# tqch/v-diffusion-torch

Measured on AMD Instinct MI355X. Metric: train_images_per_sec, higher is better.
Workload: dtype fp32 (bf16x3 split products in the tile-engine GEMMs)

## Files before the change

### include/vdiff_hip.h

```cpp
#ifndef VDIFF_HIP_H
#define VDIFF_HIP_H
#include <stddef.h>
#include <stdint.h>

#ifdef __cplusplus
extern "C" {
#endif

#define VD_VERSION 100

int         vd_version(void);
const char* vd_last_error(void);

int         vd_set_reserved_cus(int32_t n);
int         vd_reserved_cus(void);

int         vd_mfma_calibrate(float* sink, unsigned long long* stamps, int32_t blocks, int32_t iters, uint32_t seed, void* stream);

enum { VD_ROW = 0,
       VD_COL = 1,
       VD_IM2COL = 2 };

typedef struct vd_gemm_desc {
    const float* A; const float* B; float* C;
    const float* bias;
    const float* R;
    int32_t M, N, K;
    int32_t a_kind, b_kind;
    int64_t lda, ldb, ldc, ldr;
    int32_t batch, nh;
    int64_t sAb, sAh, sBb, sBh, sCb, sCh, sRb, sRh;
    float   alpha;
    int32_t accumulate;
    int32_t H, W, Cin;
    int32_t splitk;
    float*  ws; int64_t ws_bytes;
    int32_t tile;
    float*  colsum;
    int32_t colsum_accumulate;
    float*  stats;
    int32_t stats_hw;
    int64_t sBias;
} vd_gemm_desc;

int vd_gemm(const vd_gemm_desc* d, void* stream);
int vd_gemm_last_tile(void);
int vd_gemm_split_forms(void);
int vd_gemm_plan_tile(int32_t M, int32_t N, int32_t K, int32_t a_kind, int32_t b_kind, int32_t batch, int32_t tile, int32_t stats);
size_t vd_gemm_grouped_wgrad_ws_bytes(int32_t count, int32_t M, int32_t N, int32_t splitk);
int vd_gemm_grouped_wgrad_auto_split(int32_t count, int32_t M, int32_t N, int32_t K, int32_t min_slabs, int32_t max_slabs);
int vd_gemm_grouped_wgrad(const float* const* A, const float* const* B, float* const* C, float* const* colsum, int32_t count,
                          int32_t M, int32_t N, int32_t K, int64_t lda, int64_t ldb, int64_t ldc, int32_t splitk, float* ws, size_t ws_bytes,
                          void* stream);

int vd_conv3x3(const float* xin, int64_t ldx, const float* wpack, const float* bias,
               const float* res, int64_t ldres, float* y, int64_t ldy,
               int32_t nimg, int32_t H, int32_t W, int32_t Cin, int32_t Cout, int32_t accumulate,
               float* stats_part , void* stream);

int vd_conv3x3_wino_supported(int32_t nimg, int32_t H, int32_t W, int32_t Cin, int32_t Cout, int64_t ldx, int64_t ldy, int64_t ldres);
int vd_conv3x3_wino(const float* xin, int64_t ldx, const float* U, const float* bias, const float* res, int64_t ldres,
                    float* y, int64_t ldy, int32_t nimg, int32_t H, int32_t W, int32_t Cin, int32_t Cout,
                    float* stats_part, void* stream);
int vd_conv3x3_wgrad_wino_supported(int32_t nimg, int32_t H, int32_t W, int32_t Cin, int32_t Cout, int64_t ldx, int64_t lddy);
size_t vd_conv3x3_wgrad_wino_ws_bytes(int32_t nimg, int32_t H, int32_t W, int32_t Cin, int32_t Cout);
int vd_conv3x3_wgrad_wino(const float* xin, int64_t ldx, const float* dy, int64_t lddy, int32_t nimg, int32_t H, int32_t W,
                          int32_t Cin, int32_t Cout, float* dw_oihw, float* dbias, int32_t Cin_w, int32_t Cout_w,
                          int32_t accumulate, float* ws, size_t ws_bytes, void* stream);
int vd_conv3x3_wgrad_wino_phase(const float* xin, int64_t ldx, const float* dy, int64_t lddy, int32_t nimg, int32_t H, int32_t W,
                                int32_t Cin, int32_t Cout, float* dw_oihw, float* dbias, int32_t Cin_w, int32_t Cout_w,
                                int32_t accumulate, float* ws, size_t ws_bytes, int32_t phase, void* stream);
int vd_wino_last_kernel(void);
int vd_wino_wgrad_last_kernel(void);
#ifdef VD_PROBES
int vd_wino_set_probe(unsigned long long* buf);
int vd_wino43_set_probe(unsigned long long* buf);
int vd_gn_set_spin_probe(unsigned* buf);
#endif
int vd_wino_pack(const float* w_oihw, int32_t Cout, int32_t Cin, float* uf , float* ud , void* stream);
int vd_conv3x3_dgrad_wino43_supported(int32_t nimg, int32_t H, int32_t W, int32_t Cin, int32_t Cout, int64_t lddy, int64_t lddx);
size_t vd_wino43_u_floats(int32_t Cout, int32_t Cin);
int vd_conv3x3_dgrad_wino43(const float* dy, int64_t lddy, const float* U43, float* dx, int64_t lddx, int32_t nimg, int32_t H, int32_t W,
                            int32_t Cin, int32_t Cout, void* stream);
int vd_wino43_last_kernel(void);
int vd_wino43_pack(const float* w_oihw, int32_t Cout, int32_t Cin, float* U43, void* stream);
int vd_wino43_pack_batched(const int64_t* items_dev, int32_t n, int64_t total_blocks, void* stream);
int vd_conv3x3_wino43_preferred(int32_t nimg, int32_t H, int32_t W, int32_t N);
int vd_conv3x3_wino43_fwd_supported(int32_t nimg, int32_t H, int32_t W, int32_t Cin, int32_t Cout, int64_t ldx, int64_t ldy, int64_t ldres);
int vd_wino43_pack_fwd(const float* w_oihw, int32_t Cout, int32_t Cin, float* U43f, void* stream);
int vd_conv3x3_wino43_fwd_chunk_rows(int32_t H, int32_t W);
int vd_conv3x3_wino43_fwd(const float* xin, int64_t ldx, const float* U43f, const float* bias, const float* res, int64_t ldres, float* y,
                          int64_t ldy, int32_t nimg, int32_t H, int32_t W, int32_t Cin, int32_t Cout, float* stats_part, void* stream);
int vd_conv3x3_wgrad_wino43_supported(int32_t nimg, int32_t H, int32_t W, int32_t Cin, int32_t Cout, int64_t ldx, int64_t lddy);
size_t vd_conv3x3_wgrad_wino43_ws_bytes(int32_t nimg, int32_t H, int32_t W, int32_t Cin, int32_t Cout);
int vd_conv3x3_wgrad_wino43(const float* xin, int64_t ldx, const float* dy, int64_t lddy, int32_t nimg, int32_t H, int32_t W,
                            int32_t Cin, int32_t Cout, float* dw_oihw, float* dbias, int32_t Cin_w, int32_t Cout_w,
                            int32_t accumulate, float* ws, size_t ws_bytes, void* stream);
int vd_conv3x3_wgrad_wino43_phase(const float* xin, int64_t ldx, const float* dy, int64_t lddy, int32_t nimg, int32_t H, int32_t W,
                                  int32_t Cin, int32_t Cout, float* dw_oihw, float* dbias, int32_t Cin_w, int32_t Cout_w,
                                  int32_t accumulate, float* ws, size_t ws_bytes, int32_t phase, void* stream);
int vd_wino43_wgrad_last_kernel(void);

int vd_wino_pack_batched(const int64_t* items_dev, int32_t n, int64_t total_blocks, void* stream);

int vd_im2col3x3(const float* x, int64_t ldx, float* xc , int32_t nimg, int32_t H, int32_t W, int32_t C, void* stream);
int vd_tap_gather(const float* z, int64_t ldz, const float* bias, float* out, int64_t ldo, int32_t nimg, int32_t H, int32_t W, int32_t Cout, void* stream);
int vd_tap_spread(const float* dy, int64_t lddy, float* dz, int64_t ldz, int32_t nimg, int32_t H, int32_t W, int32_t Cout, void* stream);
int vd_thin_wgrad_finish(const float* g, int32_t Cout_w, int32_t Cin, int32_t Cin_w, float* dw_oihw, int32_t accumulate,
                         const float* colsum, int32_t cs_stride, int32_t cs_off, float* dbias, void* stream);

size_t vd_conv3x3_wgrad_ws_bytes(int32_t nimg, int32_t H, int32_t W, int32_t Cin, int32_t Cout);
int vd_conv3x3_wgrad(const float* xin, int64_t ldx, const float* dy, int64_t lddy,
                     int32_t nimg, int32_t H, int32_t W, int32_t Cin, int32_t Cout,
                     float* dw_oihw, float* dbias, int32_t Cin_w, int32_t Cout_w, int32_t accumulate,
                     float* ws, size_t ws_bytes, void* stream);
int vd_conv3x3_wgrad_phase(const float* xin, int64_t ldx, const float* dy, int64_t lddy,
                           int32_t nimg, int32_t H, int32_t W, int32_t Cin, int32_t Cout,
                           float* dw_oihw, float* dbias, int32_t Cin_w, int32_t Cout_w, int32_t accumulate,
                           float* ws, size_t ws_bytes, int32_t phase, void* stream);

int vd_pack_conv3x3(const float* w_oihw, int32_t Cout_w, int32_t Cin_w,
                    float* wf, int32_t Cin_p, float* wd, int32_t Cout_p, void* stream);
int vd_pack_conv3x3_batched(const int64_t* items_dev, int32_t n, int64_t total_blocks, void* stream);

enum { VD_RS_NONE = 0, VD_RS_DOWN = 1, VD_RS_UP = 2 };

size_t vd_gn_ws_bytes(int32_t nimg, int32_t HW, int32_t C);
int vd_gn_stats(const float* x, int64_t ldx, int32_t nimg, int32_t HW, int32_t C, int32_t G, float eps,
                float* stats, float* ws, size_t ws_bytes, void* stream);

int vd_gn_stats_from_partials(const float* part1, int32_t C1, int32_t chunks1, const float* part2, int32_t C2, int32_t chunks2,
                              int32_t nimg, int32_t HW, int32_t G, float eps, float* stats, void* stream);

int vd_gn_coef_from_partials(const float* part1, int32_t C1, int32_t chunks1, const float* part2, int32_t C2, int32_t chunks2,
                             int32_t nimg, int32_t HW, int32_t G, float eps, const float* gamma, const float* beta,
                             const float* film, float* coef, void* stream);

int vd_gn_apply(const float* x, int64_t ldx, const float* stats, const float* gamma, const float* beta,
                const float* film, int32_t act, float p_drop, uint64_t seed,
                int32_t resample, float* y, int64_t ldy,
                int32_t nimg, int32_t H, int32_t W, int32_t C, int32_t G, float* coef, void* stream);

int vd_gn_apply_from_partials(const float* x, int64_t ldx, const float* part1, int32_t C1, int32_t chunks1, const float* part2, int32_t C2,
                              int32_t chunks2, const float* gamma, const float* beta, const float* film, int32_t act, float p_drop,
                              uint64_t seed, int32_t resample, float* y, int64_t ldy, int32_t nimg, int32_t H, int32_t W, int32_t C,
                              int32_t G, float eps, float* coef, void* stream);

int vd_gn_apply_bwd(const float* dy, int64_t lddy, const float* x, int64_t ldx, const float* coef,
                    const float* gamma, const float* beta, const float* film, int32_t act, float p_drop, uint64_t seed,
                    int32_t resample, const float* add, int64_t ldadd, float* dx, int64_t lddx, int32_t accumulate_dx,
                    float* dfilm, float* dgamma, float* dbeta, int32_t accumulate_params,
                    int32_t nimg, int32_t H, int32_t W, int32_t C, int32_t G,
                    float* ws, size_t ws_bytes, void* stream);
int vd_gn_bwd_last_kernel(void);
int vd_gn_apply_bwd_keep(const float* dy, int64_t lddy, const float* x, int64_t ldx, const float* coef, const float* gamma,
                         const float* beta, const float* film, int32_t act, float p_drop, uint64_t seed, int32_t resample,
                         const float* add, int64_t ldadd, float* dx, int64_t lddx, int32_t accumulate_dx, float* dfilm, float* pgb_keep,
                         int32_t nimg, int32_t H, int32_t W, int32_t C, int32_t G, float* ws, size_t ws_bytes, void* stream);
int vd_gn_param_sums_batched(const int64_t* items_dev, int32_t n, int64_t total_blocks, void* stream);

size_t vd_colsum_ws_bytes(int64_t M, int32_t N);
int vd_colsum(const float* x, int64_t ldx, int64_t M, int32_t N, float* out, int32_t accumulate,
              float* ws, size_t ws_bytes, void* stream);
int vd_axpby(const float* x, int64_t ldx, float alpha, float* y, int64_t ldy, float beta, int64_t rows, int32_t C, void* stream);
int vd_silu(const float* x, float* y, int64_t n, void* stream);
int vd_silu_bwd(const float* x, const float* dy, float* dx, int64_t n, int32_t accumulate, void* stream);
int vd_softmax_rows(float* s, int64_t rows, int32_t L, void* stream);
int vd_softmax_rows_bwd(const float* p, float* dp, int64_t rows, int32_t L, float alpha, void* stream);

int vd_attn_supported(int32_t L, int32_t hd, int32_t backward);
int vd_attn_fwd(const float* q, const float* k, const float* v, int64_t ld, float* o, int64_t ldo, float* lse, int32_t B,
                int32_t nh, int32_t L, int32_t hd, float scale, void* stream);
int vd_attn_bwd(const float* q, const float* k, const float* v, int64_t ld, const float* o, int64_t ldo, const float* dout,
                int64_t lddo, const float* lse, float* delta, float* dq, float* dk, float* dv, int64_t ldd, int32_t B,
                int32_t nh, int32_t L, int32_t hd, float scale, void* stream);
int vd_attn_bwd_phase(const float* q, const float* k, const float* v, int64_t ld, const float* o, int64_t ldo, const float* dout,
                      int64_t lddo, const float* lse, float* delta, float* dq, float* dk, float* dv, int64_t ldd, int32_t B,
                      int32_t nh, int32_t L, int32_t hd, float scale, int32_t phase, void* stream);

int vd_nchw_to_nhwc(const float* x, float* y, int32_t nimg, int32_t C, int32_t H, int32_t W, int64_t ldy, void* stream);
int vd_nhwc_to_nchw(const float* x, int64_t ldx, float* y, int32_t nimg, int32_t C, int32_t H, int32_t W, void* stream);

int vd_images_to_uint8_hwc(const float* x_nchw, uint8_t* out_hwc, int32_t n, int32_t C, int32_t HW, void* stream);
int vd_images_from_uint8_hwc(const uint8_t* in_hwc, const uint8_t* flip, float* out_nchw, int32_t n, int32_t C,
// ... 114 lines not shown
```

### v-diffusion-torch_amd/csrc/common.h

```cpp
#pragma once
#include <hip/hip_runtime.h>
#include <stdint.h>
#include <stdio.h>
#include "../../include/vdiff_hip.h"

typedef float f32x4 __attribute__((ext_vector_type(4)));
typedef float f32x16 __attribute__((ext_vector_type(16)));

typedef float f32x2 __attribute__((ext_vector_type(2)));

#ifdef VD_PROBES
constexpr bool VD_PROBE_BUILD = true;
#else
constexpr bool VD_PROBE_BUILD = false;
#endif

void vd_set_error(const char* fmt, ...);
int vd_cu_count(void);
int vd_persistent_cus(void);
int vd_gemm_grouped_wgrad_kblk(const float* const* A, const float* const* B, float* const* C, float* const* colsum, int32_t count, int32_t M,
                               int32_t N, int32_t K, int64_t lda, int64_t ldb, int64_t ldc, int32_t splitk, float* ws, size_t ws_bytes,
                               void* stream, int64_t a_kblk, int64_t b_kblk, int32_t slabs_only);
int vd_gemm_grouped_wgrad_used_slabs(int32_t count, int32_t M, int32_t N, int32_t K, int32_t splitk);
extern thread_local int vd_g_last_tile;
inline int vd_tile_code(bool tr, bool spl, int kt, int bm, int bn) {
    return ((((tr ? 1 : 0) + (spl ? 2 : 0)) * 100 + kt) * 1000 + bm) * 1000 + bn;
}

#define VD_REQUIRE(cond, ...)                                   \
    do { if (!(cond)) { vd_set_error(__VA_ARGS__); return 1; } } while (0)

#define VD_LAUNCH_CHECK(name)                                                            \
    do { hipError_t e_ = hipGetLastError();                                              \
         if (e_ != hipSuccess) { vd_set_error("%s: %s", name, hipGetErrorString(e_)); return 2; } } while (0)

static inline bool vd_aligned16(const void* p) { return (reinterpret_cast<uintptr_t>(p) & 15) == 0; }

__device__ __forceinline__ float vd_sigmoid(float x) { return __builtin_amdgcn_rcpf(1.0f + __expf(-x)); }

__device__ __forceinline__ void vd_philox4(uint64_t seed, uint64_t ctr, uint32_t out[4]) {
    uint32_t k0 = (uint32_t)seed, k1 = (uint32_t)(seed >> 32);
    uint32_t c0 = (uint32_t)ctr, c1 = (uint32_t)(ctr >> 32), c2 = 0x243F6A88u, c3 = 0x85A308D3u;
#pragma unroll
    for (int r = 0; r < 10; ++r) {
        uint64_t p0 = (uint64_t)0xD2511F53u * c0, p1 = (uint64_t)0xCD9E8D57u * c2;
        uint32_t n0 = (uint32_t)(p1 >> 32) ^ c1 ^ k0, n2 = (uint32_t)(p0 >> 32) ^ c3 ^ k1;
        c1 = (uint32_t)p1; c3 = (uint32_t)p0; c0 = n0; c2 = n2;
        k0 += 0x9E3779B9u; k1 += 0xBB67AE85u;
    }
    out[0] = c0; out[1] = c1; out[2] = c2; out[3] = c3;
}
__device__ __forceinline__ f32x4 vd_dropout_scale4(uint64_t seed, uint64_t vec_index, float p) {
    uint32_t r[4];
    vd_philox4(seed, vec_index, r);
    const float inv = 1.0f / (1.0f - p);
    f32x4 m;
#pragma unroll
    for (int j = 0; j < 4; ++j) m[j] = ((r[j] >> 8) * (1.0f / 16777216.0f) >= p) ? inv : 0.0f;
    return m;
}
```

### v-diffusion-torch_amd/csrc/gemm.hip

```cpp
#include "common.h"
#include <math.h>
#include <stdlib.h>
#include <type_traits>

namespace {

constexpr int KT = 32;
#ifndef VD_GEMM_SPLIT_DEFAULT
#define VD_GEMM_SPLIT_DEFAULT 1
#endif

struct GemmArgs {
    const float* A; const float* B; float* C; const float* bias; const float* R;
    int M, N, K;
    long long lda, ldb, ldc, ldr;
    int nh;
    long long sAb, sAh, sBb, sBh, sCb, sCh, sRb, sRh;
    float alpha; int accumulate;
    int H, W, Cin;
    int kt_total, kt_per_split;
    long long slab_stride;
    float* colsum; int colsum_accumulate;
    int probe;
    float* stats; int stats_hw;
// ... 343 lines not shown
__device__ __forceinline__ void gemm_dma_body(const GemmArgs& p, const std::conditional_t<GROUPED, GroupPtrs, NoGroup>& gp) {
    constexpr int NBUF = 2;
    __shared__ __attribute__((aligned(1024))) float smem[NBUF * (BM + BN) * KT];
    constexpr int MT = BM / 64, NT = BN / 64;
    constexpr int AIT = BM * KT / 1024, BIT = BN * KT / 1024;
    constexpr int A_LPR = BM / 4, B_LPR = BN / 4;
    constexpr int A_RPP = 64 / A_LPR, B_RPP = 64 / B_LPR;
    constexpr int RLPR = KT / 4, RRPP = 64 / RLPR;
    constexpr bool A2 = (AK == VD_COL) && (MT == 2);
    constexpr bool B2 = (BK != VD_ROW) && (NT == 2 || NT == 4);
    typedef float f32x2 __attribute__((ext_vector_type(2)));
    typedef std::conditional_t<NT == 4, f32x4, f32x2> f32xNT;
    static_assert(NT <= 2 || (SPL && KT == 16 && !SPLITK && !GROUPED && AK != VD_IM2COL && BK != VD_IM2COL),
                  "256-column tiles: split-operand KT = 16 forms of plain / batched launches only");

    const int tid = threadIdx.x, lane = tid & 63;
    const int wave = __builtin_amdgcn_readfirstlane(tid >> 6);
    const int li = lane & 31, lh = lane >> 5;
    const int wm = (wave >> 1) * (BM / 2), wn = (wave & 1) * (BN / 2);
    int tbx = blockIdx.x, tby = blockIdx.y, tbz = blockIdx.z;
    {
        const unsigned T = gridDim.x * gridDim.y * gridDim.z;
        const unsigned lin = (blockIdx.z * gridDim.y + blockIdx.y) * gridDim.x + blockIdx.x;
        if (T >= 16) {
            const unsigned q = T / 8, r = T % 8, xcd = lin % 8, slot = lin / 8;
            const unsigned t = (xcd < r ? xcd * (q + 1) : r * (q + 1) + (xcd - r) * q) + slot;
            tbx = t % gridDim.x; tby = (t / gridDim.x) % gridDim.y; tbz = t / (gridDim.x * gridDim.y);
        }
    }
    const int m0 = tby * BM;
    int n0 = tbx * BN;
    int tapN = 0, ci0 = 0;
    if (BK == VD_IM2COL) {
        const int cchN = (p.Cin + BN - 1) / BN;
        tapN = tbx / cchN;
        ci0 = (tbx % cchN) * BN;
        n0 = tapN * p.Cin + ci0;
    }
    const float* A = p.A;
    const float* B = p.B;
    float* C = p.C;
    const float* R = p.R;
    const float* biasp = p.bias;
    int kt_begin = 0, kt_end = p.kt_total;
    if (SPLITK) {
        int slab = tbz;
        if constexpr (GROUPED) {
            const int e = tbz / p.group_S;
            slab = tbz - e * p.group_S;
            A = gp.A[e];
            B = gp.B[e];
        }
        kt_begin = slab * p.kt_per_split;
        kt_end = min(kt_begin + p.kt_per_split, p.kt_total);
        C += (long long)tbz * p.slab_stride;
    } else {
        const int zb = tbz / p.nh, zh = tbz % p.nh;
        A += zb * p.sAb + zh * p.sAh;
        B += zb * p.sBb + zh * p.sBh;
        C += zb * p.sCb + zh * p.sCh;
        if (R) R += zb * p.sRb + zh * p.sRh;
        if (biasp) biasp += zb * p.sBias;
    }

    unsigned voA[AIT], voB[BIT];
    unsigned mkA[AIT];
    int kcA[AIT], kcB[BIT];
    int by[BIT], bx[BIT];
    int tapA = (AK == VD_IM2COL) ? kt_begin % 9 : 0, ccA = (AK == VD_IM2COL) ? kt_begin / 9 : 0;
    const int kinc_x = (BK == VD_IM2COL) ? KT % p.W : 0, kinc_y = (BK == VD_IM2COL) ? KT / p.W : 0;
#pragma unroll
    for (int j = 0; j < AIT; ++j) {
        const int q = j * 4 + wave;
        if (AK == VD_COL) {
            const int kk = q * A_RPP + lane / A_LPR, cm = (lane % A_LPR) * 4;
            const int rowoff = (GROUPED && p.a_kblk) ? (kk >> 4) * (int)p.a_kblk + (kk & 15) * (int)p.lda : kk * (int)p.lda;
            voA[j] = (m0 + cm < p.M) ? (unsigned)(rowoff + cm) * 4u : OOB;
            kcA[j] = kk; mkA[j] = 0;
        } else {
            const int row = q * RRPP + lane / RLPR;
            const int c = (lane % RLPR) ^ swz_of<KT>(row);
            const int m = m0 + row;
            kcA[j] = c * 4;
            voA[j] = (m < p.M) ? (unsigned)(row * (int)p.lda + c * 4) * 4u : OOB;
            unsigned mk = 0;
            if (AK == VD_IM2COL) {
                int y, x;
                pix_yx(p, m, y, x);
                const unsigned xm = (x > 0 ? 1u : 0u) | 2u | (x < p.W - 1 ? 4u : 0u);
                mk = (y > 0 ? xm : 0u) | (xm << 3) | (y < p.H - 1 ? xm << 6 : 0u);
            }
            mkA[j] = mk;
        }
    }
#pragma unroll
    for (int j = 0; j < BIT; ++j) {
        const int q = j * 4 + wave;
        if (BK == VD_ROW) {
            const int row = q * RRPP + lane / RLPR;
            const int c = (lane % RLPR) ^ swz_of<KT>(row);
            kcB[j] = c * 4;
            voB[j] = (n0 + row < p.N) ? (unsigned)(row * (int)p.ldb + c * 4) * 4u : OOB;
            by[j] = bx[j] = 0;
        } else {
            const int kk = q * B_RPP + lane / B_LPR, cn = (lane % B_LPR) * 4;
            kcB[j] = kk;
            const bool ok = (BK == VD_IM2COL) ? (ci0 + cn < p.Cin) : (n0 + cn < p.N);
            const int rowoff = (GROUPED && BK == VD_COL && p.b_kblk) ? (kk >> 4) * (int)p.b_kblk + (kk & 15) * (int)p.ldb : kk * (int)p.ldb;
            voB[j] = ok ? (unsigned)(rowoff + cn) * 4u : OOB;
            if (BK == VD_IM2COL) pix_yx(p, kt_begin * KT + kk, by[j], bx[j]);
            else by[j] = bx[j] = 0;
        }
    }
    const float* Ablk = (AK == VD_COL) ? A + m0 : A + (long long)m0 * p.lda;
    const float* Bblk = (BK == VD_ROW) ? B + (long long)n0 * p.ldb : ((BK == VD_COL) ? B + n0 : B + ci0);
    const long long tapoffB = (BK == VD_IM2COL) ? (long long)((tapN / 3 - 1) * p.W + (tapN % 3 - 1)) * p.ldb : 0;

#ifndef VD_ISSUE_IN
#define VD_ISSUE_IN 2
#endif
    constexpr bool ISSUE_IN = VD_ISSUE_IN == 2 ? (AK == VD_COL) : (VD_ISSUE_IN == 1);
    struct Prep { const float* pA; const float* pB; unsigned vA[AIT], vB[BIT]; };
    auto prep_tiles = [&](int kt, Prep& P) {
        {
            const int tap = tapA, c0 = ccA * KT;
            long long aoff;
            int kwidth;
            if (AK == VD_IM2COL) { aoff = (long long)((tap / 3 - 1) * p.W + (tap % 3 - 1)) * p.lda + c0; kwidth = p.Cin - c0; }
            else if (AK == VD_ROW) { aoff = (long long)kt * KT; kwidth = p.K - kt * KT; }
            else { aoff = (GROUPED && p.a_kblk) ? (long long)kt * (KT / 16) * p.a_kblk : (long long)kt * KT * p.lda; kwidth = p.K - kt * KT; }
            P.pA = Ablk + aoff;
#pragma unroll
            for (int j = 0; j < AIT; ++j) {
                unsigned vo = voA[j];
                if (kcA[j] >= kwidth) vo = OOB;
                if (AK == VD_IM2COL && !((mkA[j] >> tap) & 1u)) vo = OOB;
                P.vA[j] = vo;
            }
        }
        {
            long long boff;
            int kwidth;
            if (BK == VD_ROW) {
                if (AK == VD_IM2COL) { boff = (long long)tapA * p.Cin + ccA * KT; kwidth = p.Cin - ccA * KT; }
                else { boff = (long long)kt * KT; kwidth = p.K - kt * KT; }
            } else { boff = ((GROUPED && BK == VD_COL && p.b_kblk) ? (long long)kt * (KT / 16) * p.b_kblk : (long long)kt * KT * p.ldb) + tapoffB; kwidth = p.K - kt * KT; }
            P.pB = Bblk + boff;
            const int dy = tapN / 3 - 1, dx = tapN % 3 - 1;
            if (BK == VD_IM2COL && p.lgW >= 0) {
#pragma unroll
                for (int j = 0; j < BIT; ++j) {
                    const int k0 = kt * KT + (j * 4 + wave) * B_RPP;
                    unsigned long long lanes = 0;
#pragma unroll
                    for (int u = 0; u < B_RPP; ++u) {
                        const int k = k0 + u;
                        const int rem = k & ((1 << p.lgHW) - 1), y = (rem >> p.lgW) + dy, x = (rem & ((1 << p.lgW) - 1)) + dx;
                        const bool ok = k < p.K && (unsigned)y < (unsigned)p.H && (unsigned)x < (unsigned)p.W;
                        lanes |= ok ? (((B_LPR == 64 ? 0ull : (1ull << (B_LPR & 63))) - 1ull) << (u * (B_LPR & 63))) : 0ull;
                    }
                    unsigned vo;
                    const unsigned oob = OOB;
                    asm("v_cndmask_b32 %0, %1, %2, %3" : "=v"(vo) : "v"(oob), "v"(voB[j]), "s"(lanes));
                    P.vB[j] = vo;
                }
            } else
#pragma unroll
            for (int j = 0; j < BIT; ++j) {
                unsigned vo = voB[j];
                if (kcB[j] >= kwidth) vo = OOB;
                if (BK == VD_IM2COL) {
                    if ((unsigned)(by[j] + dy) >= (unsigned)p.H || (unsigned)(bx[j] + dx) >= (unsigned)p.W) vo = OOB;
                    int nx = bx[j] + kinc_x, ny = by[j] + kinc_y;
                    if (nx >= p.W) { nx -= p.W; ++ny; }
                    while (ny >= p.H) ny -= p.H;
                    bx[j] = nx; by[j] = ny;
                }
                P.vB[j] = vo;
            }
        }
        if (AK == VD_IM2COL) { if (++tapA == 9) { tapA = 0; ++ccA; } }
    };
    auto issue_tiles = [&](int buf, const Prep& P) {
        float* as = smem + buf * (BM * KT);
        float* bs = smem + NBUF * BM * KT + buf * (BN * KT);
        const __amdgpu_buffer_rsrc_t rsA = make_rsrc(P.pA, PB(p) & 1 ? 0 : (int)OOB);
        const __amdgpu_buffer_rsrc_t rsB = make_rsrc(P.pB, PB(p) & 2 ? 0 : (int)OOB);
#pragma unroll
        for (int j = 0; j < AIT; ++j)
            __builtin_amdgcn_raw_ptr_buffer_load_lds(rsA, (lds_ptr_t)(as + (j * 4 + wave) * 256), 16, (int)P.vA[j], 0, 0, 0);
#pragma unroll
        for (int j = 0; j < BIT; ++j)
            __builtin_amdgcn_raw_ptr_buffer_load_lds(rsB, (lds_ptr_t)(bs + (j * 4 + wave) * 256), 16, (int)P.vB[j], 0, 0, 0);
    };

    f32x16 acc[MT][NT];
#pragma unroll
// ... 674 lines not shown
    else hipLaunchKernelGGL((gemm_dma_kernel<BM, BN, AK, BK, SPLITK, KTV, TR, GROUPED>), grid, dim3(256), 0, st, a, gp);
}
template <bool SPL, int BM, int BN, int AK, int BK, bool SPLITK, int KT16>
void launch_k16_tr(const GemmArgs& a, dim3 grid, hipStream_t st, bool k16, bool tr) {
    if (k16 && tr) launch_dma<SPL, BM, BN, AK, BK, SPLITK, KT16, true, false>(a, NoGroup{}, grid, st);
    else if (k16) launch_dma<SPL, BM, BN, AK, BK, SPLITK, KT16, false, false>(a, NoGroup{}, grid, st);
    else if (tr) launch_dma<SPL, BM, BN, AK, BK, SPLITK, 32, true, false>(a, NoGroup{}, grid, st);
    else launch_dma<SPL, BM, BN, AK, BK, SPLITK, 32, false, false>(a, NoGroup{}, grid, st);
}

constexpr int TILE_WIDE = 128256;
static bool wide_on() {
    static const bool on = !(getenv("VD_GEMM_BN256") && atoi(getenv("VD_GEMM_BN256")) == 0);
    return on;
}
bool wide_in_range(const GemmArgs& a) {
    const long long lim = 0x70000000LL / 4;
    return 256LL * a.lda + 256 < lim && 256LL * a.ldb + 256 < lim && 128LL * a.ldc + 256 < lim && 128LL * a.ldr + 256 < lim;
}

struct GemmPlan { int tile; bool wide; int bm, bn; long long nm, nn; int ktile; bool k16, spl; };
int plan_gemm(const GemmArgs& a, int ak, int bk, int batch, int splitk, int requested, GemmPlan* out) {
    static const char* env = getenv("VD_GEMM_TILE");
    const int forced = (env && requested == 0) ? atoi(env) : requested;
    const bool conv = ak == VD_IM2COL, wgrad = bk == VD_IM2COL, want_wide = forced == TILE_WIDE;
    GemmPlan P;
    P.tile = want_wide ? 0 : choose_tile(a.M, wgrad ? a.Cin : a.N, wgrad, (long long)batch * splitk, forced);
    P.bm = TILES[P.tile].bm; P.bn = TILES[P.tile].bn;
    P.nm = (a.M + P.bm - 1) / P.bm;
    P.nn = wgrad ? 9LL * ((a.Cin + P.bn - 1) / P.bn) : (a.N + P.bn - 1) / P.bn;
    P.ktile = ktile_for(a, P.tile, P.nm * P.nn * batch, splitk > 1, wgrad && (long long)a.K >= WGRAD_WIDE_PIXELS, wgrad && splitk <= 1);
    P.k16 = P.tile == 0 && !(wgrad && splitk <= 1) && P.ktile == 16;
    P.spl = P.bm == 128 && !conv && !wgrad && use_dma(a) && split_forms();
    const bool kinds = (ak == VD_ROW && (bk == VD_ROW || bk == VD_COL)) || (ak == VD_COL && bk == VD_COL);
    const bool can = P.spl && P.tile == 0 && splitk <= 1 && kinds && a.N % 256 == 0 && wide_in_range(a);
    VD_REQUIRE(requested != TILE_WIDE || can, "vd_gemm: tile = %d needs the split-operand forms, N %% 256 == 0 (N=%d), ROW/ROW, ROW/COL or COL/COL operands "
               "and no split-K", TILE_WIDE, a.N);
    const bool natural = forced == 0 && wide_on() && ak == VD_ROW && bk == VD_ROW && P.k16 && P.nm * (a.N / 256) * batch >= 2LL * vd_cu_count();
    P.wide = can && (want_wide || natural);
    if (P.wide) { P.bn = 256; P.nn = a.N / 256; P.ktile = 16; P.k16 = true; }
    *out = P;
    return 0;
}
bool plan_tr(const GemmArgs& a, bool wgrad) { return use_dma(a) && use_tr(a, wgrad); }
int plan_code(const GemmArgs& a, const GemmPlan& P, bool tr) { return vd_tile_code(tr, P.spl, use_dma(a) ? (P.k16 ? 16 : 32) : 0, P.bm, P.bn); }

template <int AK, int BK>
void launch_wide(const GemmArgs& a, const GemmPlan& P, dim3 grid, hipStream_t st) {
    const bool tr = plan_tr(a, false);
    vd_g_last_tile = plan_code(a, P, tr);
    if (tr) launch_dma<true, 128, 256, AK, BK, false, 16, true, false>(a, NoGroup{}, grid, st);
    else launch_dma<true, 128, 256, AK, BK, false, 16, false, false>(a, NoGroup{}, grid, st);
}

template <int BM, int BN, int AK, int BK, bool SPLITK>
void launch(const GemmArgs& a, dim3 grid, hipStream_t st, const GemmPlan& P) {
    constexpr bool has16 = BM == 128 && BN == 128 && !(BK == VD_IM2COL && !SPLITK);
    constexpr bool has_spl = BM == 128 && AK != VD_IM2COL && BK != VD_IM2COL;
    const bool k16 = has16 && P.k16;
    const bool tr = plan_tr(a, BK == VD_IM2COL);
    const bool spl = has_spl && P.spl;
    vd_g_last_tile = plan_code(a, P, tr);
    if constexpr (has_spl) {
        if (spl) return launch_k16_tr<true, BM, BN, AK, BK, SPLITK, (has16 ? 16 : 32)>(a, grid, st, k16, tr);
    }
    if (!use_dma(a)) hipLaunchKernelGGL((gemm_kernel<BM, BN, AK, BK, SPLITK>), grid, dim3(256), 0, st, a);
    else launch_k16_tr<false, BM, BN, AK, BK, SPLITK, (has16 ? 16 : 32)>(a, grid, st, k16, tr);
}

template <int AK, int BK, bool SPLITK>
void launch_tile2(const GemmPlan& P, const GemmArgs& a, dim3 grid, hipStream_t st) {
    if (P.tile == 0) launch<128, 128, AK, BK, SPLITK>(a, grid, st, P);
    else if (P.tile == 1) launch<128, 64, AK, BK, SPLITK>(a, grid, st, P);
    else if (P.tile == 2) launch<64, 128, AK, BK, SPLITK>(a, grid, st, P);
    else launch<64, 64, AK, BK, SPLITK>(a, grid, st, P);
}

template <int AK, int BK>
void launch_tile(const GemmPlan& P, bool splitk, const GemmArgs& a, dim3 grid, hipStream_t st) {
    if (splitk) launch_tile2<AK, BK, true>(P, a, grid, st);
    else launch_tile2<AK, BK, false>(P, a, grid, st);
}

int run_gemm(const vd_gemm_desc& d, hipStream_t st) {
    VD_REQUIRE(d.M > 0 && d.N > 0 && d.K > 0, "vd_gemm: empty problem M=%d N=%d K=%d", d.M, d.N, d.K);
    VD_REQUIRE(d.A && d.B && d.C, "vd_gemm: null operand");
    VD_REQUIRE(vd_aligned16(d.A) && vd_aligned16(d.B), "vd_gemm: A/B must be 16-byte aligned");
    VD_REQUIRE(d.lda % 4 == 0 && d.ldb % 4 == 0, "vd_gemm: lda/ldb must be multiples of 4 floats (lda=%lld ldb=%lld)",
               (long long)d.lda, (long long)d.ldb);
    const int ak = d.a_kind, bk = d.b_kind;
    const bool conv = (ak == VD_IM2COL), wgrad = (bk == VD_IM2COL);
    VD_REQUIRE(!(conv && bk != VD_ROW), "vd_gemm: IM2COL A needs ROW B");
    VD_REQUIRE(!(wgrad && ak != VD_COL), "vd_gemm: IM2COL B needs COL A");
    if (ak == VD_ROW) VD_REQUIRE(d.K % 4 == 0, "vd_gemm: K %% 4 != 0 for k-contiguous A (K=%d)", d.K);
    if (ak == VD_COL) VD_REQUIRE(d.M % 4 == 0, "vd_gemm: M %% 4 != 0 for m-contiguous A (M=%d)", d.M);
    if (bk == VD_COL) VD_REQUIRE(d.N % 4 == 0, "vd_gemm: N %% 4 != 0 for n-contiguous B (N=%d)", d.N);
    if (conv || wgrad) VD_REQUIRE(d.Cin % 4 == 0 && d.H > 0 && d.W > 0, "vd_gemm: bad image geometry");
    const int batch = d.batch > 0 ? d.batch : 1;
    const int splitk = d.splitk > 1 ? d.splitk : 1;
    VD_REQUIRE(!(splitk > 1 && batch > 1), "vd_gemm: split-K and batch are exclusive");
    VD_REQUIRE(!(splitk > 1 && (d.bias || d.R)), "vd_gemm: split-K does not take bias/residual");

    GemmArgs a;
    a.A = d.A; a.B = d.B; a.C = d.C; a.bias = d.bias; a.R = d.R;
    a.M = d.M; a.N = d.N; a.K = d.K;
    a.lda = d.lda; a.ldb = d.ldb; a.ldc = d.ldc; a.ldr = d.ldr;
    a.nh = d.nh > 0 ? d.nh : 1;
    a.sAb = d.sAb; a.sAh = d.sAh; a.sBb = d.sBb; a.sBh = d.sBh; a.sCb = d.sCb; a.sCh = d.sCh; a.sRb = d.sRb; a.sRh = d.sRh;
    a.alpha = d.alpha; a.accumulate = d.accumulate;
    a.H = d.H; a.W = d.W; a.Cin = d.Cin;
    a.kt_total = 0; a.kt_per_split = 0; a.slab_stride = 0;
    a.colsum = d.colsum; a.colsum_accumulate = d.colsum_accumulate;
    a.stats = d.stats; a.stats_hw = d.stats_hw;
    a.sBias = d.sBias;
    a.lgW = a.lgHW = -1;
    if ((conv || wgrad) && (d.W & (d.W - 1)) == 0 && ((d.H * d.W) & (d.H * d.W - 1)) == 0) {
        a.lgW = __builtin_ctz((unsigned)d.W); a.lgHW = __builtin_ctz((unsigned)(d.H * d.W));
    }
    a.probe = 0;
#ifdef VD_PROBES
    { static const char* e = getenv("VD_GEMM_PROBE"); a.probe = e ? atoi(e) : 0; }
#endif
    VD_REQUIRE((a.probe & 16) || !(d.colsum && (ak != VD_COL || batch > 1)), "vd_gemm: colsum needs a COL-kind A operand and batch 1");

    GemmPlan P;
    if (plan_gemm(a, ak, bk, batch, splitk, d.tile, &P)) return 1;
    const int tbm = P.bm;
    const long long nm = P.nm, nn = P.nn;
    VD_REQUIRE(nm <= 65535, "vd_gemm: too many row tiles (%lld)", nm);
    if (d.stats && !(a.probe & 32)) {
        VD_REQUIRE(batch == 1 && splitk == 1 && !wgrad && bk == VD_ROW && ak != VD_COL, "vd_gemm: output statistics need a plain forward launch");
        VD_REQUIRE(d.stats_hw > 0 && d.stats_hw % (tbm / 2) == 0 && d.M % d.stats_hw == 0,
                   "vd_gemm: output statistics need H*W (%d) to be a multiple of half the row tile (%d)", d.stats_hw, tbm / 2);
    }
    const int ktile = P.ktile;
    a.kt_total = conv ? 9 * ((d.Cin + ktile - 1) / ktile) : (d.K + ktile - 1) / ktile;
    a.kt_per_split = a.kt_total;

    float* final_C = d.C;
    if (splitk > 1) {
        a.kt_per_split = (a.kt_total + splitk - 1) / splitk;
        const int used = (a.kt_total + a.kt_per_split - 1) / a.kt_per_split;
        a.slab_stride = (long long)d.M * d.N;
        VD_REQUIRE(d.ws && d.ws_bytes >= (int64_t)((used * a.slab_stride + (d.colsum ? (long long)used * d.M : 0)) * 4),
                   "vd_gemm: split-K workspace too small");
        a.C = d.ws; a.ldc = d.N;
        float* cpart = d.ws + used * a.slab_stride;
        if (d.colsum && !(a.probe & 16)) a.colsum = cpart;
        dim3 grid(nn, nm, used);
        if (ak == VD_COL && bk == VD_COL) launch_tile<VD_COL, VD_COL>(P, true, a, grid, st);
        else if (ak == VD_COL && bk == VD_IM2COL) launch_tile<VD_COL, VD_IM2COL>(P, true, a, grid, st);
        else if (ak == VD_ROW && bk == VD_ROW) launch_tile<VD_ROW, VD_ROW>(P, true, a, grid, st);
        else if (ak == VD_ROW && bk == VD_COL) launch_tile<VD_ROW, VD_COL>(P, true, a, grid, st);
        else VD_REQUIRE(false, "vd_gemm: split-K not built for kinds (%d,%d)", ak, bk);
        VD_LAUNCH_CHECK("gemm_kernel(splitk)");
        if (!wgrad && !(a.probe & 16)) {
            const long long tot = (long long)d.M * d.N;
            hipLaunchKernelGGL(reduce_slabs_kernel, dim3((tot + 255) / 256), dim3(256), 0, st, d.ws, used, a.slab_stride,
                               d.M, d.N, final_C, d.ldc, d.accumulate, d.alpha, cpart, d.colsum, d.colsum_accumulate);
            VD_LAUNCH_CHECK("reduce_slabs_kernel");
        }
        return 0;
    }
    dim3 grid(nn, nm, batch);
    if (P.wide) {
        if (ak == VD_ROW && bk == VD_ROW) launch_wide<VD_ROW, VD_ROW>(a, P, grid, st);
        else if (ak == VD_ROW) launch_wide<VD_ROW, VD_COL>(a, P, grid, st);
        else launch_wide<VD_COL, VD_COL>(a, P, grid, st);
        VD_LAUNCH_CHECK("gemm_split_kernel(128x256)");
        return 0;
    }
    if (ak == VD_ROW && bk == VD_ROW) launch_tile<VD_ROW, VD_ROW>(P, false, a, grid, st);
    else if (ak == VD_ROW && bk == VD_COL) launch_tile<VD_ROW, VD_COL>(P, false, a, grid, st);
    else if (ak == VD_COL && bk == VD_COL) launch_tile<VD_COL, VD_COL>(P, false, a, grid, st);
    else if (ak == VD_COL && bk == VD_ROW) launch_tile<VD_COL, VD_ROW>(P, false, a, grid, st);
    else if (ak == VD_IM2COL && bk == VD_ROW) launch_tile<VD_IM2COL, VD_ROW>(P, false, a, grid, st);
    else if (ak == VD_COL && bk == VD_IM2COL) launch_tile<VD_COL, VD_IM2COL>(P, false, a, grid, st);
    else VD_REQUIRE(false, "vd_gemm: unsupported operand kinds (%d,%d)", ak, bk);
    VD_LAUNCH_CHECK("gemm_kernel");
    return 0;
}

template <int BM, int BN, int KTV = 32>
void launch_grouped(const GemmArgs& a, const GroupPtrs& gp, dim3 grid, hipStream_t st) {
    const bool spl = split_forms();
    vd_g_last_tile = vd_tile_code(true, spl, KTV, BM, BN);
    if (spl) launch_dma<true, BM, BN, VD_COL, VD_COL, true, KTV, true, true>(a, gp, grid, st);
    else launch_dma<false, BM, BN, VD_COL, VD_COL, true, KTV, true, true>(a, gp, grid, st);
}
constexpr long long GROUPED_K16_MIN_WGS = 768;
static bool planes256(int count, int M, int N, int K) {
    static const bool on = !(getenv("VD_PLANES256") && atoi(getenv("VD_PLANES256")) == 0);
    if (!(on && split_forms() && M % 256 == 0 && N % 256 == 0 && K % 16 == 0)) return false;
    const long long blocks = (long long)(M / 256) * (N / 256) * count, slots = vd_cu_count();
    const int kmax = K / 256 > 1 ? K / 256 : 1;
    double best = 0.0;
    for (int sl = 1; sl <= 24 && sl <= kmax; ++sl) {
// ... 52 lines not shown
extern "C" int vd_gemm_grouped_wgrad(const float* const* A, const float* const* B, float* const* C, float* const* colsum, int32_t count,
                                     int32_t M, int32_t N, int32_t K, int64_t lda, int64_t ldb, int64_t ldc, int32_t splitk, float* ws,
                                     size_t ws_bytes, void* stream) {
    return vd_gemm_grouped_wgrad_kblk(A, B, C, colsum, count, M, N, K, lda, ldb, ldc, splitk, ws, ws_bytes, stream, 0, 0, 0);
}

int vd_gemm_grouped_wgrad_used_slabs(int32_t count, int32_t M, int32_t N, int32_t K, int32_t splitk) {
    return plan_grouped(count, M, N, K, splitk > 1 ? splitk : 1).used;
}

int vd_gemm_grouped_wgrad_kblk(const float* const* A, const float* const* B, float* const* C, float* const* colsum, int32_t count,
                               int32_t M, int32_t N, int32_t K, int64_t lda, int64_t ldb, int64_t ldc, int32_t splitk, float* ws,
                               size_t ws_bytes, void* stream, int64_t a_kblk, int64_t b_kblk, int32_t slabs_only) {
    VD_REQUIRE(A && B && C && count > 0 && count <= VD_GROUP_MAX, "vd_gemm_grouped_wgrad: 1..%d entries (got %d)", VD_GROUP_MAX, count);
    VD_REQUIRE(M > 0 && N > 0 && K > 0 && M % 4 == 0 && N % 4 == 0 && lda % 4 == 0 && ldb % 4 == 0 && ldc >= N,
               "vd_gemm_grouped_wgrad: M, N, lda, ldb must be multiples of 4 (M=%d N=%d)", M, N);
    const int S = splitk > 1 ? splitk : 1;
    VD_REQUIRE(ws && ws_bytes >= vd_gemm_grouped_wgrad_ws_bytes(count, M, N, S), "vd_gemm_grouped_wgrad: workspace too small");
    GemmArgs a = {};
    GroupPtrs gp = {};
    GroupOut go = {};
    for (int e = 0; e < count; ++e) {
        VD_REQUIRE(A[e] && B[e] && C[e] && vd_aligned16(A[e]) && vd_aligned16(B[e]), "vd_gemm_grouped_wgrad: entry %d: null / unaligned operand", e);
        gp.A[e] = A[e]; gp.B[e] = B[e]; go.C[e] = C[e]; go.cs[e] = colsum ? colsum[e] : nullptr;
    }
    a.A = A[0]; a.B = B[0];
    a.M = M; a.N = N; a.K = K; a.lda = lda; a.ldb = ldb; a.ldc = N; a.ldr = 0; a.nh = 1;
    a.alpha = 1.f; a.lgW = a.lgHW = -1; a.probe = 0;
    a.a_kblk = a_kblk; a.b_kblk = b_kblk;
    VD_REQUIRE(a_kblk >= 0 && b_kblk >= 0 && a_kblk % 4 == 0 && b_kblk % 4 == 0 && 2 * a_kblk + 16 * lda + 128 < 0x70000000LL / 4 &&
               2 * b_kblk + 16 * ldb + 128 < 0x70000000LL / 4, "vd_gemm_grouped_wgrad: K-block strides outside the LDS-DMA kernel's range");
    VD_REQUIRE(dma_in_range(a), "vd_gemm_grouped_wgrad: operands outside the LDS-DMA kernel's range (alignment / row pitch)");
    const GroupedPlan g = plan_grouped(count, M, N, K, S);
    const int used = g.used;
    a.kt_total = g.kt_total; a.kt_per_split = g.kt_per_split; a.group_S = used;
    a.slab_stride = (long long)M * N;
    a.C = ws;
    float* cpart = ws + (long long)count * used * a.slab_stride;
    a.colsum = colsum ? cpart : nullptr;
    const dim3 grid((unsigned)g.nn, (unsigned)g.nm, (unsigned)(count * used));
    hipStream_t st = (hipStream_t)stream;
    if (g.p256) {
        vd_g_last_tile = vd_tile_code(true, true, 16, 256, 256);
        hipLaunchKernelGGL(wgrad_planes256_kernel, grid, dim3(512), 0, st, a, gp);
    } else if (g.tile == 0 && g.k16) launch_grouped<128, 128, 16>(a, gp, grid, st);
    else if (g.tile == 0) launch_grouped<128, 128>(a, gp, grid, st);
    else if (g.tile == 1) launch_grouped<128, 64>(a, gp, grid, st);
    else if (g.tile == 2) launch_grouped<64, 128>(a, gp, grid, st);
    else launch_grouped<64, 64>(a, gp, grid, st);
    VD_LAUNCH_CHECK("gemm_dma_kernel(grouped)");
    if (slabs_only) return 0;
    const long long tot = (long long)M * N;
    hipLaunchKernelGGL(reduce_slabs_grouped_kernel, dim3((unsigned)((tot + 255) / 256), (unsigned)count), dim3(256), 0, st, ws, used,
                       a.slab_stride, M, N, go, (long long)ldc, cpart);
    VD_LAUNCH_CHECK("reduce_slabs_grouped_kernel");
    return 0;
}

thread_local int vd_g_last_tile = 0;
extern "C" int vd_gemm_last_tile(void) { return vd_g_last_tile; }

extern "C" int vd_gemm_plan_tile(int32_t M, int32_t N, int32_t K, int32_t a_kind, int32_t b_kind, int32_t batch, int32_t tile, int32_t stats) {
    if (!(M > 0 && N > 0 && K > 0 && a_kind >= VD_ROW && a_kind <= VD_COL && b_kind >= VD_ROW && b_kind <= VD_COL)) {
        vd_set_error("vd_gemm_plan_tile: plain operand kinds and a non-empty problem only");
        return -1;
    }
    float* const aligned = reinterpret_cast<float*>(uintptr_t(4096));
    GemmArgs a = {};
    a.A = a.B = aligned; a.C = aligned;
    a.M = M; a.N = N; a.K = K;
    a.lda = a_kind == VD_ROW ? K : M; a.ldb = b_kind == VD_ROW ? K : N; a.ldc = N;
    a.nh = 1; a.alpha = 1.f; a.lgW = a.lgHW = -1;
    a.stats = stats ? aligned : nullptr;
    GemmPlan P;
    if (plan_gemm(a, a_kind, b_kind, batch > 0 ? batch : 1, 1, tile, &P)) return -1;
    return plan_code(a, P, plan_tr(a, false));
}

extern "C" int vd_gemm(const vd_gemm_desc* d, void* stream) {
    VD_REQUIRE(d != nullptr, "vd_gemm: null descriptor");
    return run_gemm(*d, (hipStream_t)stream);
}

extern "C" int vd_conv3x3(const float* xin, int64_t ldx, const float* wpack, const float* bias, const float* res,
                          int64_t ldres, float* y, int64_t ldy, int32_t nimg, int32_t H, int32_t W, int32_t Cin,
                          int32_t Cout, int32_t accumulate, float* stats_part, void* stream) {
    VD_REQUIRE(Cin % 4 == 0, "vd_conv3x3: Cin must be a multiple of 4 (got %d)", Cin);
    vd_gemm_desc d = {};
    d.A = xin; d.B = wpack; d.C = y; d.bias = bias; d.R = res;
    d.M = nimg * H * W; d.N = Cout; d.K = 9 * Cin;
    d.a_kind = VD_IM2COL; d.b_kind = VD_ROW;
    d.lda = ldx; d.ldb = 9LL * Cin; d.ldc = ldy; d.ldr = ldres;
    d.batch = 1; d.nh = 1; d.alpha = 1.f; d.accumulate = accumulate;
    d.H = H; d.W = W; d.Cin = Cin;
    d.stats = stats_part; d.stats_hw = H * W;
    if (stats_part && (H * W) % 64 != 0) d.tile = 64;
    return run_gemm(d, (hipStream_t)stream);
}

static void wgrad_plan(int nimg, int H, int W, int Cin, int Cout, int* tile_out, int* split_out) {
    const int t = choose_tile(Cout, Cin, true, 64, 0);
    const long long kt = ((long long)nimg * H * W + 31) / 32;
    const long long tiles = ((Cout + TILES[t].bm - 1) / TILES[t].bm) * 9LL * ((Cin + TILES[t].bn - 1) / TILES[t].bn);
    const bool wide = t == 0 && (long long)nimg * H * W >= WGRAD_WIDE_PIXELS;
    const long long slots = 256LL * (wide ? 4 : TILES[t].per_cu);
    int best = 1;
    double best_eff = 0.0;
    for (int s = 1; s <= 64; ++s) {
        if (s > 1 && kt / s < 16) break;
        const long long blocks = tiles * s;
        const long long rounds = (blocks + slots - 1) / slots;
        double eff = (double)blocks / (double)(rounds * slots);
        eff *= 1.0 - 0.004 * s;
        if (eff > best_eff) { best_eff = eff; best = s; }
    }
    *tile_out = t; *split_out = best;
}

extern "C" size_t vd_conv3x3_wgrad_ws_bytes(int32_t nimg, int32_t H, int32_t W, int32_t Cin, int32_t Cout) {
    int t, S;
    wgrad_plan(nimg, H, W, Cin, Cout, &t, &S);
    return (size_t)S * ((size_t)Cout * 9 * Cin + Cout) * sizeof(float);
}

static int conv3x3_wgrad_impl(const float* xin, int64_t ldx, const float* dy, int64_t lddy, int32_t nimg, int32_t H, int32_t W,
                              int32_t Cin, int32_t Cout, float* dw_oihw, float* dbias, int32_t Cin_w, int32_t Cout_w,
                              int32_t accumulate, float* ws, size_t ws_bytes, hipStream_t st, int phases) {
    VD_REQUIRE(Cin % 4 == 0 && Cout % 4 == 0, "vd_conv3x3_wgrad: Cin/Cout must be multiples of 4 (%d,%d)", Cin, Cout);
    VD_REQUIRE(Cin_w <= Cin && Cout_w <= Cout, "vd_conv3x3_wgrad: real dims exceed padded dims");
    int t, S;
    wgrad_plan(nimg, H, W, Cin, Cout, &t, &S);
    static const int codes[4] = {128, 12864, 64128, 64};
    VD_REQUIRE(ws && ws_bytes >= (size_t)S * ((size_t)Cout * 9 * Cin + Cout) * 4, "vd_conv3x3_wgrad: workspace too small");
    const long long slab = (long long)Cout * 9 * Cin;
    int used = 1;
    if (S > 1) {
        GemmArgs ga = {};
        ga.A = dy; ga.B = xin; ga.lda = lddy; ga.ldb = ldx; ga.ldc = 9LL * Cin; ga.ldr = 0;
        const long long K = (long long)nimg * H * W;
        const int ktile = ktile_for(ga, t, 0, true, K >= WGRAD_WIDE_PIXELS);
        const long long kt_total = (K + ktile - 1) / ktile, per = (kt_total + S - 1) / S;
        used = (int)((kt_total + per - 1) / per);
    }
    if (phases & 1) {
        vd_gemm_desc d = {};
        d.A = dy; d.B = xin; d.C = ws;
        d.M = Cout; d.N = 9 * Cin; d.K = nimg * H * W;
        d.a_kind = VD_COL; d.b_kind = VD_IM2COL;
        d.lda = lddy; d.ldb = ldx; d.ldc = 9LL * Cin;
        d.batch = 1; d.nh = 1; d.alpha = 1.f;
        d.H = H; d.W = W; d.Cin = Cin;
        d.splitk = S; d.ws = ws; d.ws_bytes = (int64_t)ws_bytes; d.tile = codes[t];
        if (S > 1) {
            d.colsum = dbias;
        } else {
            d.splitk = 1;
            d.colsum = dbias ? ws + slab : nullptr; d.colsum_accumulate = 0;
        }
        int rc = run_gemm(d, st);
        if (rc) return rc;
    }
    if (phases & 2) {
        float* cpart = ws + used * slab;
        hipLaunchKernelGGL(reduce_slabs_oihw_kernel, dim3((slab + 255) / 256), dim3(256), 0, st, ws, used, slab, Cout, Cin,
                           Cout_w, Cin_w, dw_oihw, accumulate, cpart, dbias);
        VD_LAUNCH_CHECK("reduce_slabs_oihw_kernel");
// ... 40 lines not shown
```

### v-diffusion-torch_amd/csrc/wino43.hip

```cpp
#include "common.h"
#include <type_traits>

namespace {

typedef __attribute__((address_space(3))) void* lds_ptr_t;
constexpr unsigned OOB = 0x80000000u;
constexpr int KT = 8;
constexpr int TN = 32;
constexpr int TILES = 64;
constexpr int U_STAGE = 36 * 4 * 16 * 2 * 2;
constexpr int THREADS = 512;

struct Args43 {
    const float* x; long long ldx;
    const float* U;
    float* y; long long ldy;
    int nimg, H, W, K, N;
    int items_per_img;
    int ngrp;
    int ncb, nitems;
    const float* bias; const float* res; long long ldr;
    float* stats;
    int chunks_per_img;
    unsigned long long* probe;
};

__device__ __forceinline__ void lds_barrier() { asm volatile("s_waitcnt lgkmcnt(0)\n\ts_barrier" ::: "memory"); }

__device__ __forceinline__ __amdgpu_buffer_rsrc_t make_rsrc(const float* base, int records = (int)OOB) {
    return __builtin_amdgcn_make_buffer_rsrc((void*)base, 0, records, 0x00020000);
}

constexpr int SB_STEP = 12;
constexpr int U_AHEAD = 2;
template <int HALF, bool DY, typename T>
__device__ __forceinline__ void bt_half(const T (&d)[6], T& o0, T& o1, T& o2) {
    if (DY) {
        if (HALF == 0) {
            const T e1 = d[4] - 2.25f * d[2], f1 = d[3] - 2.25f * d[1];
            o0 = 1.265625f * d[0] + (d[4] - 2.8125f * d[2]);
            o1 = e1 + 0.75f * f1;
            o2 = e1 - 0.75f * f1;
        } else {
            const T e2 = d[4] - 0.5625f * d[2], f2 = d[3] - 0.5625f * d[1];
            o0 = e2 + 1.5f * f2;
            o1 = e2 - 1.5f * f2;
            o2 = 1.265625f * d[1] + (d[5] - 2.8125f * d[3]);
        }
    } else if (HALF == 0) {
        const T t = d[4] - 4.f * d[2], u = d[3] - 4.f * d[1];
        o0 = 4.f * d[0] + (d[4] - 5.f * d[2]);
        o1 = t + u;
        o2 = t - u;
    } else {
        const T c = d[4] - d[2], e = d[3] - d[1];
        o0 = c + 2.f * e;
        o1 = c - 2.f * e;
        o2 = 4.f * d[1] + (d[5] - 5.f * d[3]);
    }
}
template <bool DY, typename T>
__device__ __forceinline__ void bt_full(const T (&r)[6], T (&v)[6]) {
    if (DY) {
        const T e1 = r[4] - 2.25f * r[2], f1 = r[3] - 2.25f * r[1];
        const T e2 = r[4] - 0.5625f * r[2], f2 = r[3] - 0.5625f * r[1];
        v[0] = 1.265625f * r[0] + (r[4] - 2.8125f * r[2]);
        v[1] = e1 + 0.75f * f1;
        v[2] = e1 - 0.75f * f1;
        v[3] = e2 + 1.5f * f2;
        v[4] = e2 - 1.5f * f2;
        v[5] = 1.265625f * r[1] + (r[5] - 2.8125f * r[3]);
        return;
    }
    const T t = r[4] - 4.f * r[2], u = r[3] - 4.f * r[1], c = r[4] - r[2], e = r[3] - r[1];
    v[0] = 4.f * r[0] + (r[4] - 5.f * r[2]);
    v[1] = t + u;
    v[2] = t - u;
    v[3] = c + 2.f * e;
    v[4] = c - 2.f * e;
    v[5] = 4.f * r[1] + (r[5] - 5.f * r[3]);
}
template <int HALF, bool DY>
__device__ __forceinline__ void bt_half2(const f32x2 (&d)[6], f32x2& o0, f32x2& o1, f32x2& o2) { bt_half<HALF, DY, f32x2>(d, o0, o1, o2); }
// ... 349 lines not shown
            cb = cb_next; grp = grp_next; have = have_next;
        }
    };
    if ((wave >> 2) == 0) run(std::integral_constant<int, 0>{});
    else run(std::integral_constant<int, 1>{});
}

__device__ __forceinline__ void pack43_tile(const float* w, float* U, int Cout, int Cin, int tile, int fwd) {
    const int nkt = (fwd ? Cin : Cout) / KT;
    const int nb = tile / nkt, kt = tile - nb * nkt;
    const int t = threadIdx.x;
    const int kq = t >> 6, n = (t >> 2) & 15, cbk = (t >> 1) & 1, j = t & 1;
    const int cn = nb * 32 + 16 * cbk + n, ck = kt * KT + 2 * kq + j;
    const int ci = fwd ? ck : cn, co = fwd ? cn : ck;
    const float* src = w + ((long long)co * Cin + ci) * 9;
    double g[3][3];
#pragma unroll
    for (int a = 0; a < 3; ++a)
#pragma unroll
        for (int b = 0; b < 3; ++b) g[a][b] = (double)(fwd ? src[a * 3 + b] : src[(2 - a) * 3 + (2 - b)]);
    const double Gc[6][3] = {{0.25, 0.0, 0.0}, {-1.0 / 6, -1.0 / 6, -1.0 / 6}, {-1.0 / 6, 1.0 / 6, -1.0 / 6},
                             {1.0 / 24, 1.0 / 12, 1.0 / 6}, {1.0 / 24, -1.0 / 12, 1.0 / 6}, {0.0, 0.0, 1.0}};
    const double Gd[6][3] = {{64.0 / 81, 0.0, 0.0}, {-128.0 / 243, -32.0 / 81, -8.0 / 27}, {-128.0 / 243, 32.0 / 81, -8.0 / 27},
                             {32.0 / 243, 16.0 / 81, 8.0 / 27}, {32.0 / 243, -16.0 / 81, 8.0 / 27}, {0.0, 0.0, 1.0}};
    double Gm[6][3];
#pragma unroll
    for (int a = 0; a < 6; ++a)
#pragma unroll
        for (int c = 0; c < 3; ++c) Gm[a][c] = fwd ? Gd[a][c] : Gc[a][c];
    double tmp[6][3];
#pragma unroll
    for (int a = 0; a < 6; ++a)
#pragma unroll
        for (int c = 0; c < 3; ++c) tmp[a][c] = Gm[a][0] * g[0][c] + Gm[a][1] * g[1][c] + Gm[a][2] * g[2][c];
    float* dst = U + ((long long)nb * nkt + kt) * U_STAGE + t;
#pragma unroll
    for (int a = 0; a < 6; ++a)
#pragma unroll
        for (int b = 0; b < 6; ++b)
            dst[(6 * a + b) * 256] = (float)(tmp[a][0] * Gm[b][0] + tmp[a][1] * Gm[b][1] + tmp[a][2] * Gm[b][2]);
}

__global__ __launch_bounds__(256) void wino43_pack_kernel(const float* w, float* U, int Cout, int Cin, int fwd) {
    pack43_tile(w, U, Cout, Cin, blockIdx.x, fwd);
}

__global__ __launch_bounds__(256) void wino43_pack_batched_kernel(const long long* items, int n) {
    int lo = 0, hi = n - 1;
    while (lo < hi) {
        const int mid = (lo + hi + 1) >> 1;
        if (items[8 * mid + 7] <= (long long)blockIdx.x) lo = mid; else hi = mid - 1;
    }
    const long long* it = items + 8 * lo;
    pack43_tile(reinterpret_cast<const float*>(it[0]), reinterpret_cast<float*>(it[1]), (int)it[3], (int)it[4],
                (int)((long long)blockIdx.x - it[7]), (int)it[2]);
}

__device__ __forceinline__ void bt6(const f32x4 (&d)[6], f32x4 (&o)[6]) {
    const f32x4 e1 = d[4] - 2.25f * d[2], f1 = 0.75f * d[3] - 1.6875f * d[1];
    const f32x4 e2 = d[4] - 0.5625f * d[2], f2 = 1.5f * d[3] - 0.84375f * d[1];
    o[0] = 1.265625f * d[0] + (d[4] - 2.8125f * d[2]);
    o[1] = e1 + f1;
    o[2] = e1 - f1;
    o[3] = e2 + f2;
    o[4] = e2 - f2;
    o[5] = 1.265625f * d[1] + (d[5] - 2.8125f * d[3]);
}
__device__ __forceinline__ void a6(const f32x4 (&y)[4], f32x4 (&o)[6]) {
    const f32x4 e1 = y[0] + 0.5625f * y[2], f1 = 0.75f * y[1] + 0.421875f * y[3];
    const f32x4 e2 = y[0] + 2.25f * y[2], f2 = 1.5f * y[1] + 3.375f * y[3];
    o[0] = y[0];
    o[1] = e1 + f1;
    o[2] = e1 - f1;
    o[3] = e2 + f2;
    o[4] = e2 - f2;
    o[5] = y[3];
}

__device__ __forceinline__ void st_once(float* p, f32x4 v) { *reinterpret_cast<f32x4*>(p) = v; }
struct WgT43 {
    const float* x; long long ldx; const float* dy; long long lddy;
    float* V; float* dM;
    int nimg, H, W, Cin, Cout, TW, TPI, T;
};

__global__ __launch_bounds__(256) void wino43_wgrad_transform_kernel(const WgT43 p) {
    const int quad = blockIdx.y * 64 + threadIdx.x, tile = blockIdx.x * 4 + threadIdx.y;
    if (tile >= p.T) return;
    const int img = tile / p.TPI, tin = tile - img * p.TPI;
    const int ty = tin / p.TW, tx = tin - ty * p.TW;
    const int c4 = 4 * quad;
    if (blockIdx.z == 0) {
        if (c4 >= p.Cin) return;
        f32x4 R[6][6];
#pragma unroll
        for (int pr = 0; pr < 6; ++pr) {
            const int yy = 4 * ty - 1 + pr;
            f32x4 d[6];
#pragma unroll
            for (int q = 0; q < 6; ++q) {
                const int xx = 4 * tx - 1 + q;
                d[q] = f32x4{0.f, 0.f, 0.f, 0.f};
                if ((unsigned)yy < (unsigned)p.H && (unsigned)xx < (unsigned)p.W)
                    d[q] = *reinterpret_cast<const f32x4*>(p.x + ((long long)(img * p.H + yy) * p.W + xx) * p.ldx + c4);
            }
            bt6(d, R[pr]);
        }
#pragma unroll
        for (int b = 0; b < 6; ++b) {
            f32x4 col[6], o[6];
#pragma unroll
            for (int pr = 0; pr < 6; ++pr) col[pr] = R[pr][b];
            bt6(col, o);
#pragma unroll
            for (int a = 0; a < 6; ++a)
                st_once(p.V + ((long long)((tile >> 4) * 36 + 6 * a + b) * 16 + (tile & 15)) * p.Cin + c4, o[a]);
        }
    } else {
        if (c4 >= p.Cout) return;
        f32x4 R[4][6];
#pragma unroll
        for (int u = 0; u < 4; ++u) {
            f32x4 y[4];
#pragma unroll
            for (int v = 0; v < 4; ++v)
                y[v] = *reinterpret_cast<const f32x4*>(p.dy + ((long long)(img * p.H + 4 * ty + u) * p.W + 4 * tx + v) * p.lddy + c4);
            a6(y, R[u]);
        }
#pragma unroll
        for (int b = 0; b < 6; ++b) {
            const f32x4 col[4] = {R[0][b], R[1][b], R[2][b], R[3][b]};
            f32x4 o[6];
            a6(col, o);
#pragma unroll
            for (int a = 0; a < 6; ++a)
                st_once(p.dM + ((long long)((tile >> 4) * 36 + 6 * a + b) * 16 + (tile & 15)) * p.Cout + c4, o[a]);
        }
    }
}

__global__ __launch_bounds__(256) void wino43_wgrad_finish_kernel(const float* dU, const float* cs, int Cout, int Cin, int Cout_w, int Cin_w,
                                                                  float* dw, float* dbias, int accumulate) {
    const long long idx = (long long)blockIdx.x * blockDim.x + threadIdx.x;
    if (dbias && idx < Cout_w) {
        const double pv[6] = {-1.0 / 9, 8.0 / 9, 0.0, 2.0 / 9, 0.0, -1.0 / 8};
        double c = 0.0;
#pragma unroll
        for (int a = 0; a < 6; ++a)
#pragma unroll
            for (int b = 0; b < 6; ++b)
                if (pv[a] != 0.0 && pv[b] != 0.0) c += pv[a] * pv[b] * (double)cs[(long long)(6 * a + b) * Cout + idx];
        dbias[idx] = accumulate ? dbias[idx] + (float)c : (float)c;
    }
    if (idx >= (long long)Cout * Cin) return;
    const int co = (int)(idx / Cin), ci = (int)(idx - (long long)co * Cin);
    if (co >= Cout_w || ci >= Cin_w) return;
    float u[6][6];
#pragma unroll
    for (int a = 0; a < 6; ++a)
#pragma unroll
        for (int b = 0; b < 6; ++b) u[a][b] = dU[(long long)(6 * a + b) * Cout * Cin + idx];
    constexpr float g0 = 64.f / 81, g12 = 128.f / 243, g34 = 32.f / 243, h12 = 32.f / 81, h34 = 16.f / 81, k = 8.f / 27;
    float t[3][6];
#pragma unroll
    for (int b = 0; b < 6; ++b) {
        const float s12 = u[1][b] + u[2][b], d12 = u[2][b] - u[1][b], s34 = u[3][b] + u[4][b], d34 = u[3][b] - u[4][b];
        t[0][b] = g0 * u[0][b] - g12 * s12 + g34 * s34;
        t[1][b] = h12 * d12 + h34 * d34;
        t[2][b] = k * (s34 - s12) + u[5][b];
    }
    float* o = dw + ((long long)co * Cin_w + ci) * 9;
#pragma unroll
    for (int r = 0; r < 3; ++r) {
        const float s12 = t[r][1] + t[r][2], d12 = t[r][2] - t[r][1], s34 = t[r][3] + t[r][4], d34 = t[r][3] - t[r][4];
        const float w0 = g0 * t[r][0] - g12 * s12 + g34 * s34;
        const float w1 = h12 * d12 + h34 * d34;
        const float w2 = k * (s34 - s12) + t[r][5];
        o[3 * r] = accumulate ? o[3 * r] + w0 : w0;
        o[3 * r + 1] = accumulate ? o[3 * r + 1] + w1 : w1;
        o[3 * r + 2] = accumulate ? o[3 * r + 2] + w2 : w2;
    }
}

constexpr long long FUSED_FINISH_MIN = 147456;
__global__ __launch_bounds__(384) void wino43_wgrad_reduce_finish_kernel(const float* slabs, const float* cpart, int S, int Cout, int Cin,
                                                                         int Cout_w, int Cin_w, float* dw, float* dbias, int accumulate) {
    __shared__ float tsh[3][6][64];
    const int x = threadIdx.x, b = threadIdx.y;
    const long long idx = (long long)blockIdx.x * 64 + x;
    if (dbias && b == 0 && idx < Cout_w) {
        const double pv[6] = {-1.0 / 9, 8.0 / 9, 0.0, 2.0 / 9, 0.0, -1.0 / 8};
        double c = 0.0;
#pragma unroll
        for (int a = 0; a < 6; ++a)
#pragma unroll
            for (int bb = 0; bb < 6; ++bb)
                if (pv[a] != 0.0 && pv[bb] != 0.0) {
                    float cs = 0.f;
                    for (int z = 0; z < S; ++z) cs += cpart[((long long)(6 * a + bb) * S + z) * Cout + idx];
                    c += pv[a] * pv[bb] * (double)cs;
                }
        dbias[idx] = accumulate ? dbias[idx] + (float)c : (float)c;
    }
    const long long plane = (long long)Cout * Cin;
    const bool in = idx < plane;
    constexpr float g0 = 64.f / 81, g12 = 128.f / 243, g34 = 32.f / 243, h12 = 32.f / 81, h34 = 16.f / 81, k = 8.f / 27;
    {
        float u[6] = {0.f, 0.f, 0.f, 0.f, 0.f, 0.f};
        if (in) {
            const float* sl = slabs + (long long)b * S * plane + idx;
            const long long astep = 6LL * S * plane;
            for (int z = 0; z < S; ++z) {
#pragma unroll
                for (int a = 0; a < 6; ++a) u[a] += sl[a * astep + z * plane];
            }
        }
        const float s12 = u[1] + u[2], d12 = u[2] - u[1], s34 = u[3] + u[4], d34 = u[3] - u[4];
        tsh[0][b][x] = g0 * u[0] - g12 * s12 + g34 * s34;
        tsh[1][b][x] = h12 * d12 + h34 * d34;
        tsh[2][b][x] = k * (s34 - s12) + u[5];
    }
    __syncthreads();
    if (!in || b >= 3) return;
    const int co = (int)(idx / Cin), ci = (int)(idx - (long long)co * Cin);
    if (co >= Cout_w || ci >= Cin_w) return;
    const int r = b;
    float t[6];
#pragma unroll
    for (int c = 0; c < 6; ++c) t[c] = tsh[r][c][x];
    const float s12 = t[1] + t[2], d12 = t[2] - t[1], s34 = t[3] + t[4], d34 = t[3] - t[4];
    const float w0 = g0 * t[0] - g12 * s12 + g34 * s34;
    const float w1 = h12 * d12 + h34 * d34;
    const float w2 = k * (s34 - s12) + t[5];
    float* o = dw + ((long long)co * Cin_w + ci) * 9 + 3 * r;
    o[0] = accumulate ? o[0] + w0 : w0;
    o[1] = accumulate ? o[1] + w1 : w1;
    o[2] = accumulate ? o[2] + w2 : w2;
}

struct Wg43Plan { bool ok; int T, S; size_t v_f, m_f, u_f, cs_f, gemm_bytes; };
Wg43Plan wg43_plan(int nimg, int H, int W, int Cin, int Cout) {
    Wg43Plan g = {};
    if (nimg <= 0 || H % 4 || W % 4 || H < 4 || W < 4 || Cin % 4 || Cout % 4) return g;
    g.T = nimg * (H / 4) * (W / 4);
    g.S = vd_gemm_grouped_wgrad_auto_split(36, Cout, Cin, g.T, (g.T + 1535) / 1536, 24);
    const size_t T16 = ((size_t)g.T + 15) / 16 * 16;
    g.v_f = (size_t)36 * T16 * Cin; g.m_f = (size_t)36 * T16 * Cout; g.u_f = (size_t)36 * Cout * Cin; g.cs_f = (size_t)36 * Cout;
    g.gemm_bytes = vd_gemm_grouped_wgrad_ws_bytes(36, Cout, Cin, g.S);
    g.ok = true;
    return g;
}

thread_local int g_last43 = 0;
#ifdef VD_PROBES
unsigned long long* g_probe43 = nullptr;
#else
constexpr unsigned long long* g_probe43 = nullptr;
#endif
thread_local int g_last43w = 0;

}

extern "C" int vd_conv3x3_dgrad_wino43_supported(int32_t nimg, int32_t H, int32_t W, int32_t Cin, int32_t Cout, int64_t lddy, int64_t lddx) {
    if (nimg <= 0 || Cout % KT || Cin % TN || lddy % 4 || lddx % 4) return 0;
    if (!((W == 32 && H == 32) || (W == 64 && H % 16 == 0 && H >= 16) || (W == 16 && H == 16 && nimg % 4 == 0))) return 0;
    const long long px = (W == 16 ? (long long)nimg : 1LL) * H * W, lim = 0x7FFFFFF0LL / 4;
    if (px * lddy >= lim || px * lddx >= lim) return 0;
    return 1;
}

extern "C" size_t vd_wino43_u_floats(int32_t Cout, int32_t Cin) { return (size_t)36 * Cout * Cin; }

extern "C" int vd_conv3x3_wino43_preferred(int32_t nimg, int32_t H, int32_t W, int32_t N) {
    if (nimg <= 0 || N <= 0) return 0;
    const long long grp = W == 16 ? (nimg + 3) / 4 : (long long)nimg * (W == 64 ? H / 16 : 1);
    const long long i43 = grp * ((N + TN - 1) / TN), ncu = vd_persistent_cus();
    const long long r43 = (i43 + ncu - 1) / ncu, r23 = (4 * i43 + ncu - 1) / ncu;
    return 8 * r43 < 3 * r23;
}

extern "C" int vd_conv3x3_dgrad_wino43(const float* dy, int64_t lddy, const float* U43, float* dx, int64_t lddx, int32_t nimg, int32_t H,
                                       int32_t W, int32_t Cin, int32_t Cout, void* stream) {
    VD_REQUIRE(dy && U43 && dx, "vd_conv3x3_dgrad_wino43: null operand");
    VD_REQUIRE(vd_conv3x3_dgrad_wino43_supported(nimg, H, W, Cin, Cout, lddy, lddx),
               "vd_conv3x3_dgrad_wino43: unsupported geometry nimg=%d H=%d W=%d Cin=%d Cout=%d", nimg, H, W, Cin, Cout);
    VD_REQUIRE(vd_aligned16(dy) && vd_aligned16(U43) && vd_aligned16(dx), "vd_conv3x3_dgrad_wino43: operands must be 16-byte aligned");
    Args43 a = {};
    a.x = dy; a.ldx = lddy; a.U = U43; a.y = dx; a.ldy = lddx;
    a.nimg = nimg; a.H = H; a.W = W; a.K = Cout; a.N = Cin;
    a.items_per_img = W == 64 ? H / 16 : 1;
    a.ngrp = W == 16 ? nimg / 4 : nimg * a.items_per_img;
    a.ncb = Cin / TN;
    const long long items = (long long)a.ngrp * a.ncb;
    VD_REQUIRE(items < (1LL << 30), "vd_conv3x3_dgrad_wino43: too many work items");
    a.nitems = (int)items;
    a.probe = g_probe43;
    const int ncu = vd_persistent_cus();
    const dim3 grid((unsigned)(items < ncu ? items : ncu)), blk(THREADS);
    hipStream_t st = (hipStream_t)stream;
    if (W == 16) hipLaunchKernelGGL((wino43_conv_kernel<4, false>), grid, blk, 0, st, a);
    else if (W == 32) hipLaunchKernelGGL((wino43_conv_kernel<8, false>), grid, blk, 0, st, a);
    else hipLaunchKernelGGL((wino43_conv_kernel<16, false>), grid, blk, 0, st, a);
    VD_LAUNCH_CHECK("wino43_conv_kernel<., false>");
    g_last43 = W / 4;
    return 0;
}

extern "C" int vd_wino43_last_kernel(void) { return g_last43; }
#ifdef VD_PROBES
extern "C" int vd_wino43_set_probe(unsigned long long* buf) { g_probe43 = buf; return 0; }
#endif

extern "C" int vd_wino43_pack(const float* w_oihw, int32_t Cout, int32_t Cin, float* U43, void* stream) {
    VD_REQUIRE(w_oihw && U43 && Cout % KT == 0 && Cin % TN == 0, "vd_wino43_pack: needs Cout %% 8 == 0 and Cin %% 32 == 0");
    hipLaunchKernelGGL(wino43_pack_kernel, dim3((unsigned)((Cin / TN) * (Cout / KT))), dim3(256), 0, (hipStream_t)stream, w_oihw, U43, Cout, Cin, 0);
    VD_LAUNCH_CHECK("wino43_pack_kernel");
    return 0;
}

extern "C" int vd_conv3x3_wino43_fwd_supported(int32_t nimg, int32_t H, int32_t W, int32_t Cin, int32_t Cout, int64_t ldx, int64_t ldy,
                                               int64_t ldres) {
    if (nimg <= 0 || Cin % KT || Cout % TN || ldx % 4 || ldy % 4 || ldres % 4) return 0;
    if (!((W == 32 && H == 32) || (W == 64 && H % 16 == 0 && H >= 16) || (W == 16 && H == 16 && nimg % 4 == 0))) return 0;
    const long long px = (W == 16 ? (long long)nimg : 1LL) * H * W, lim = 0x7FFFFFF0LL / 4;
    if (px * ldx >= lim || px * ldy >= lim || (ldres > 0 && px * ldres >= lim)) return 0;
    return 1;
}

extern "C" int vd_wino43_pack_fwd(const float* w_oihw, int32_t Cout, int32_t Cin, float* U43f, void* stream) {
    VD_REQUIRE(w_oihw && U43f && Cin % KT == 0 && Cout % TN == 0, "vd_wino43_pack_fwd: needs Cin %% 8 == 0 and Cout %% 32 == 0");
    hipLaunchKernelGGL(wino43_pack_kernel, dim3((unsigned)((Cout / TN) * (Cin / KT))), dim3(256), 0, (hipStream_t)stream, w_oihw, U43f, Cout, Cin, 1);
    VD_LAUNCH_CHECK("wino43_pack_kernel(fwd)");
    return 0;
}

extern "C" int vd_conv3x3_wino43_fwd_chunk_rows(int32_t H, int32_t W) { return W == 16 ? H * W : (W == 32 ? H * W : 16 * W); }

extern "C" int vd_conv3x3_wino43_fwd(const float* xin, int64_t ldx, const float* U43f, const float* bias, const float* res, int64_t ldres,
                                     float* y, int64_t ldy, int32_t nimg, int32_t H, int32_t W, int32_t Cin, int32_t Cout,
                                     float* stats_part, void* stream) {
    VD_REQUIRE(xin && U43f && y, "vd_conv3x3_wino43_fwd: null operand");
    VD_REQUIRE(vd_conv3x3_wino43_fwd_supported(nimg, H, W, Cin, Cout, ldx, ldy, res ? ldres : 0),
               "vd_conv3x3_wino43_fwd: unsupported geometry nimg=%d H=%d W=%d Cin=%d Cout=%d", nimg, H, W, Cin, Cout);
    VD_REQUIRE(vd_aligned16(xin) && vd_aligned16(U43f) && vd_aligned16(y) && (!res || vd_aligned16(res)) && (!bias || vd_aligned16(bias)),
               "vd_conv3x3_wino43_fwd: operands must be 16-byte aligned");
    Args43 a = {};
    a.x = xin; a.ldx = ldx; a.U = U43f; a.y = y; a.ldy = ldy;
    a.nimg = nimg; a.H = H; a.W = W; a.K = Cin; a.N = Cout;
    a.items_per_img = W == 64 ? H / 16 : 1;
    a.ngrp = W == 16 ? nimg / 4 : nimg * a.items_per_img;
    a.ncb = Cout / TN;
    a.bias = bias; a.res = res; a.ldr = ldres; a.stats = stats_part;
    a.chunks_per_img = (H * W) / vd_conv3x3_wino43_fwd_chunk_rows(H, W);
    VD_REQUIRE(a.chunks_per_img == a.items_per_img, "vd_conv3x3_wino43_fwd: statistics chunks (%d per image) do not match the work items (%d)", a.chunks_per_img, a.items_per_img);
    const long long items = (long long)a.ngrp * a.ncb;
    VD_REQUIRE(items < (1LL << 30), "vd_conv3x3_wino43_fwd: too many work items");
    a.nitems = (int)items;
    a.probe = g_probe43;
    const int ncu = vd_persistent_cus();
    const dim3 grid((unsigned)(items < ncu ? items : ncu)), blk(THREADS);
    hipStream_t st = (hipStream_t)stream;
    if (W == 16) hipLaunchKernelGGL((wino43_conv_kernel<4, true>), grid, blk, 0, st, a);
    else if (W == 32) hipLaunchKernelGGL((wino43_conv_kernel<8, true>), grid, blk, 0, st, a);
    else hipLaunchKernelGGL((wino43_conv_kernel<16, true>), grid, blk, 0, st, a);
    VD_LAUNCH_CHECK("wino43_conv_kernel<., true>");
    g_last43 = -(W / 4);
    return 0;
}

extern "C" int vd_wino43_pack_batched(const int64_t* items_dev, int32_t n, int64_t total_blocks, void* stream) {
    VD_REQUIRE(items_dev && n > 0 && total_blocks > 0 && total_blocks < (1LL << 31), "vd_wino43_pack_batched: bad table");
    hipLaunchKernelGGL(wino43_pack_batched_kernel, dim3((unsigned)total_blocks), dim3(256), 0, (hipStream_t)stream,
                       reinterpret_cast<const long long*>(items_dev), n);
    VD_LAUNCH_CHECK("wino43_pack_batched_kernel");
    return 0;
}

extern "C" int vd_conv3x3_wgrad_wino43_supported(int32_t nimg, int32_t H, int32_t W, int32_t Cin, int32_t Cout, int64_t ldx, int64_t lddy) {
    const Wg43Plan g = wg43_plan(nimg, H, W, Cin, Cout);
    if (!g.ok || ldx % 4 || lddy % 4 || g.T < 512 || g.T % 4) return 0;
    const long long px = (long long)nimg * H * W, lim = 0x7FFFFFF0LL / 4;
    if (px * ldx >= lim || px * lddy >= lim) return 0;
    if ((long long)g.T * (Cin > Cout ? Cin : Cout) * 4 >= (1LL << 40)) return 0;
    return 1;
}

extern "C" size_t vd_conv3x3_wgrad_wino43_ws_bytes(int32_t nimg, int32_t H, int32_t W, int32_t Cin, int32_t Cout) {
    const Wg43Plan g = wg43_plan(nimg, H, W, Cin, Cout);
    if (!g.ok) return 0;
    return (g.v_f + g.m_f + g.u_f + g.cs_f) * sizeof(float) + g.gemm_bytes;
}

static int wgrad43_impl(const float* xin, int64_t ldx, const float* dy, int64_t lddy, int32_t nimg, int32_t H, int32_t W, int32_t Cin,
                        int32_t Cout, float* dw_oihw, float* dbias, int32_t Cin_w, int32_t Cout_w, int32_t accumulate, float* ws,
                        size_t ws_bytes, void* stream, int phases) {
    VD_REQUIRE(xin && dy && dw_oihw && ws, "vd_conv3x3_wgrad_wino43: null operand");
    VD_REQUIRE(vd_conv3x3_wgrad_wino43_supported(nimg, H, W, Cin, Cout, ldx, lddy),
               "vd_conv3x3_wgrad_wino43: unsupported geometry nimg=%d H=%d W=%d Cin=%d Cout=%d", nimg, H, W, Cin, Cout);
    VD_REQUIRE(Cin_w <= Cin && Cout_w <= Cout, "vd_conv3x3_wgrad_wino43: real dims exceed padded dims");
    VD_REQUIRE(vd_aligned16(xin) && vd_aligned16(dy) && vd_aligned16(ws), "vd_conv3x3_wgrad_wino43: operands must be 16-byte aligned");
    VD_REQUIRE(ws_bytes >= vd_conv3x3_wgrad_wino43_ws_bytes(nimg, H, W, Cin, Cout), "vd_conv3x3_wgrad_wino43: workspace too small");
    const Wg43Plan g = wg43_plan(nimg, H, W, Cin, Cout);
    float* V = ws;
    float* dM = V + g.v_f;
    float* dU = dM + g.m_f;
    float* cs = dU + g.u_f;
    float* gws = cs + g.cs_f;
    hipStream_t st = (hipStream_t)stream;
    if (phases & 1) {
        WgT43 t = {};
        t.x = xin; t.ldx = ldx; t.dy = dy; t.lddy = lddy; t.V = V; t.dM = dM;
        t.nimg = nimg; t.H = H; t.W = W; t.Cin = Cin; t.Cout = Cout; t.TW = W / 4; t.TPI = (H / 4) * (W / 4); t.T = g.T;
        const int cmax = Cin > Cout ? Cin : Cout;
        hipLaunchKernelGGL(wino43_wgrad_transform_kernel, dim3((unsigned)(g.T / 4), (unsigned)((cmax + 255) / 256), 2), dim3(64, 4), 0, st, t);
        VD_LAUNCH_CHECK("wino43_wgrad_transform_kernel");
    }
    if (phases & 2) {
        const float* A[36]; const float* B[36]; float* C[36]; float* colsum[36];
        for (int e = 0; e < 36; ++e) {
            A[e] = dM + (size_t)e * 16 * Cout; B[e] = V + (size_t)e * 16 * Cin;
            C[e] = dU + (size_t)e * Cout * Cin; colsum[e] = cs + (size_t)e * Cout;
        }
        const int rc = vd_gemm_grouped_wgrad_kblk(A, B, C, colsum, 36, Cout, Cin, g.T, Cout, Cin, Cin, g.S, gws, g.gemm_bytes, stream,
                                                  36LL * 16 * Cout, 36LL * 16 * Cin,
                                                  (long long)Cout * Cin >= FUSED_FINISH_MIN ? 1 : 0);
        if (rc) return rc;
        g_last43w = g.S;
    }
    if (phases & 4) {
        const long long tot = (long long)Cout * Cin;
        if (tot >= FUSED_FINISH_MIN) {
            const int used = vd_gemm_grouped_wgrad_used_slabs(36, Cout, Cin, g.T, g.S);
            hipLaunchKernelGGL(wino43_wgrad_reduce_finish_kernel, dim3((unsigned)((tot + 63) / 64)), dim3(64, 6), 0, st, gws,
                               gws + (size_t)36 * used * Cout * Cin, used, Cout, Cin, Cout_w, Cin_w, dw_oihw, dbias, accumulate);
        } else {
            hipLaunchKernelGGL(wino43_wgrad_finish_kernel, dim3((unsigned)((tot + 255) / 256)), dim3(256), 0, st, dU, cs, Cout, Cin, Cout_w, Cin_w,
                               dw_oihw, dbias, accumulate);
        }
        VD_LAUNCH_CHECK("wino43_wgrad_finish_kernel");
    }
    return 0;
}

extern "C" int vd_conv3x3_wgrad_wino43(const float* xin, int64_t ldx, const float* dy, int64_t lddy, int32_t nimg, int32_t H, int32_t W,
                                       int32_t Cin, int32_t Cout, float* dw_oihw, float* dbias, int32_t Cin_w, int32_t Cout_w,
                                       int32_t accumulate, float* ws, size_t ws_bytes, void* stream) {
    return wgrad43_impl(xin, ldx, dy, lddy, nimg, H, W, Cin, Cout, dw_oihw, dbias, Cin_w, Cout_w, accumulate, ws, ws_bytes, stream, 7);
}

extern "C" int vd_conv3x3_wgrad_wino43_phase(const float* xin, int64_t ldx, const float* dy, int64_t lddy, int32_t nimg, int32_t H,
                                             int32_t W, int32_t Cin, int32_t Cout, float* dw_oihw, float* dbias, int32_t Cin_w,
                                             int32_t Cout_w, int32_t accumulate, float* ws, size_t ws_bytes, int32_t phase, void* stream) {
    VD_REQUIRE(phase == 1 || phase == 2 || phase == 4, "vd_conv3x3_wgrad_wino43_phase: phase must be 1 (transforms), 2 (GEMMs) or 4 (reduction + finish)");
    return wgrad43_impl(xin, ldx, dy, lddy, nimg, H, W, Cin, Cout, dw_oihw, dbias, Cin_w, Cout_w, accumulate, ws, ws_bytes, stream, phase);
}

extern "C" int vd_wino43_wgrad_last_kernel(void) { return g_last43w; }
```

### v-diffusion-torch_amd/v_diffusion/_hip.py

```python
import ctypes as C
import os

import numpy as np
import torch

_HERE = os.path.dirname(os.path.abspath(__file__))
LIB_PATH = os.environ.get("VDIFF_HIP_LIB") or os.path.join(os.path.dirname(_HERE), "lib", "libvdiff_hip.so")

ROW, COL, IM2COL = 0, 1, 2
TILE_WIDE = 128256
RS_NONE, RS_DOWN, RS_UP = 0, 1, 2
OUT_TYPES = {"v": 0, "x0": 1, "eps": 2, "both": 3}
REWEIGHTS = {"constant": 0, "snr": 1, "snr_trunc": 2, "snr_1plus": 3}

_i32, _i64, _f32, _f64, _u64, _vp, _sz = C.c_int32, C.c_int64, C.c_float, C.c_double, C.c_uint64, C.c_void_p, C.c_size_t


class GemmDesc(C.Structure):
    _fields_ = [("A", _vp), ("B", _vp), ("C", _vp), ("bias", _vp), ("R", _vp),
                ("M", _i32), ("N", _i32), ("K", _i32), ("a_kind", _i32), ("b_kind", _i32),
                ("lda", _i64), ("ldb", _i64), ("ldc", _i64), ("ldr", _i64),
                ("batch", _i32), ("nh", _i32),
                ("sAb", _i64), ("sAh", _i64), ("sBb", _i64), ("sBh", _i64),
                ("sCb", _i64), ("sCh", _i64), ("sRb", _i64), ("sRh", _i64),
                ("alpha", _f32), ("accumulate", _i32), ("H", _i32), ("W", _i32), ("Cin", _i32),
                ("splitk", _i32), ("ws", _vp), ("ws_bytes", _i64), ("tile", _i32),
                ("colsum", _vp), ("colsum_accumulate", _i32), ("stats", _vp), ("stats_hw", _i32), ("sBias", _i64)]


_SIGNATURES = {
    "vd_version": (C.c_int, []),
    "vd_last_error": (C.c_char_p, []),
    "vd_set_reserved_cus": (C.c_int, [_i32]),
    "vd_reserved_cus": (C.c_int, []),
    "vd_mfma_calibrate": (C.c_int, [_vp, _vp, _i32, _i32, C.c_uint32, _vp]),
    "vd_gemm": (C.c_int, [C.POINTER(GemmDesc), _vp]),
    "vd_gemm_last_tile": (C.c_int, []),
    "vd_gemm_split_forms": (C.c_int, []),
    "vd_gemm_plan_tile": (C.c_int, [_i32, _i32, _i32, _i32, _i32, _i32, _i32, _i32]),
    "vd_gemm_grouped_wgrad_ws_bytes": (_sz, [_i32, _i32, _i32, _i32]),
    "vd_gemm_grouped_wgrad_auto_split": (C.c_int, [_i32, _i32, _i32, _i32, _i32, _i32]),
    "vd_gemm_grouped_wgrad": (C.c_int, [_vp, _vp, _vp, _vp, _i32, _i32, _i32, _i32, _i64, _i64, _i64, _i32, _vp, _sz, _vp]),
    "vd_conv3x3": (C.c_int, [_vp, _i64, _vp, _vp, _vp, _i64, _vp, _i64, _i32, _i32, _i32, _i32, _i32, _i32, _vp, _vp]),
    "vd_conv3x3_wino_supported": (C.c_int, [_i32, _i32, _i32, _i32, _i32, _i64, _i64, _i64]),
    "vd_conv3x3_wino": (C.c_int, [_vp, _i64, _vp, _vp, _vp, _i64, _vp, _i64, _i32, _i32, _i32, _i32, _i32, _vp, _vp]),
    "vd_wino_pack": (C.c_int, [_vp, _i32, _i32, _vp, _vp, _vp]),
    "vd_conv3x3_wgrad_wino_supported": (C.c_int, [_i32, _i32, _i32, _i32, _i32, _i64, _i64]),
    "vd_conv3x3_wgrad_wino_ws_bytes": (_sz, [_i32, _i32, _i32, _i32, _i32]),
    "vd_conv3x3_wgrad_wino": (C.c_int, [_vp, _i64, _vp, _i64, _i32, _i32, _i32, _i32, _i32, _vp, _vp, _i32, _i32, _i32, _vp, _sz, _vp]),
    "vd_conv3x3_wgrad_wino_phase": (C.c_int, [_vp, _i64, _vp, _i64, _i32, _i32, _i32, _i32, _i32, _vp, _vp, _i32, _i32, _i32, _vp, _sz, _i32, _vp]),
    "vd_wino_last_kernel": (C.c_int, []),
    "vd_wino_wgrad_last_kernel": (C.c_int, []),
    "vd_wino_pack_batched": (C.c_int, [_vp, _i32, _i64, _vp]),
    "vd_conv3x3_dgrad_wino43_supported": (C.c_int, [_i32, _i32, _i32, _i32, _i32, _i64, _i64]),
    "vd_wino43_u_floats": (_sz, [_i32, _i32]),
    "vd_conv3x3_dgrad_wino43": (C.c_int, [_vp, _i64, _vp, _vp, _i64, _i32, _i32, _i32, _i32, _i32, _vp]),
    "vd_wino43_last_kernel": (C.c_int, []),
    "vd_conv3x3_wino43_fwd_supported": (C.c_int, [_i32, _i32, _i32, _i32, _i32, _i64, _i64, _i64]),
    "vd_conv3x3_wino43_preferred": (C.c_int, [_i32, _i32, _i32, _i32]),
    "vd_wino43_pack_fwd": (C.c_int, [_vp, _i32, _i32, _vp, _vp]),
    "vd_conv3x3_wino43_fwd_chunk_rows": (C.c_int, [_i32, _i32]),
    "vd_conv3x3_wino43_fwd": (C.c_int, [_vp, _i64, _vp, _vp, _vp, _i64, _vp, _i64, _i32, _i32, _i32, _i32, _i32, _vp, _vp]),
    "vd_wino43_pack": (C.c_int, [_vp, _i32, _i32, _vp, _vp]),
    "vd_wino43_pack_batched": (C.c_int, [_vp, _i32, _i64, _vp]),
    "vd_conv3x3_wgrad_wino43_supported": (C.c_int, [_i32, _i32, _i32, _i32, _i32, _i64, _i64]),
    "vd_conv3x3_wgrad_wino43_ws_bytes": (_sz, [_i32, _i32, _i32, _i32, _i32]),
    "vd_conv3x3_wgrad_wino43": (C.c_int, [_vp, _i64, _vp, _i64, _i32, _i32, _i32, _i32, _i32, _vp, _vp, _i32, _i32, _i32, _vp, _sz, _vp]),
    "vd_wino43_wgrad_last_kernel": (C.c_int, []),
    "vd_conv3x3_wgrad_wino43_phase": (C.c_int, [_vp, _i64, _vp, _i64, _i32, _i32, _i32, _i32, _i32, _vp, _vp, _i32, _i32, _i32, _vp, _sz, _i32, _vp]),
    "vd_gn_stats_from_partials": (C.c_int, [_vp, _i32, _i32, _vp, _i32, _i32, _i32, _i32, _i32, _f32, _vp, _vp]),
    "vd_gn_coef_from_partials": (C.c_int, [_vp, _i32, _i32, _vp, _i32, _i32, _i32, _i32, _i32, _f32, _vp, _vp, _vp, _vp, _vp]),
    "vd_conv3x3_wgrad_ws_bytes": (_sz, [_i32, _i32, _i32, _i32, _i32]),
    "vd_conv3x3_wgrad": (C.c_int, [_vp, _i64, _vp, _i64, _i32, _i32, _i32, _i32, _i32, _vp, _vp, _i32, _i32, _i32, _vp, _sz, _vp]),
    "vd_conv3x3_wgrad_phase": (C.c_int, [_vp, _i64, _vp, _i64, _i32, _i32, _i32, _i32, _i32, _vp, _vp, _i32, _i32, _i32, _vp, _sz, _i32, _vp]),
    "vd_pack_conv3x3": (C.c_int, [_vp, _i32, _i32, _vp, _i32, _vp, _i32, _vp]),
    "vd_pack_conv3x3_batched": (C.c_int, [_vp, _i32, _i64, _vp]),
    "vd_gn_ws_bytes": (_sz, [_i32, _i32, _i32]),
    "vd_gn_stats": (C.c_int, [_vp, _i64, _i32, _i32, _i32, _i32, _f32, _vp, _vp, _sz, _vp]),
    "vd_gn_apply": (C.c_int, [_vp, _i64, _vp, _vp, _vp, _vp, _i32, _f32, _u64, _i32, _vp, _i64, _i32, _i32, _i32, _i32, _i32, _vp, _vp]),
    "vd_gn_apply_from_partials": (C.c_int, [_vp, _i64, _vp, _i32, _i32, _vp, _i32, _i32, _vp, _vp, _vp, _i32, _f32, _u64, _i32, _vp, _i64, _i32,
                                            _i32, _i32, _i32, _i32, _f32, _vp, _vp]),
    "vd_gn_apply_bwd": (C.c_int, [_vp, _i64, _vp, _i64, _vp, _vp, _vp, _vp, _i32, _f32, _u64, _i32, _vp, _i64, _vp, _i64, _i32,
                                  _vp, _vp, _vp, _i32, _i32, _i32, _i32, _i32, _i32, _vp, _sz, _vp]),
    "vd_gn_bwd_last_kernel": (C.c_int, []),
    "vd_gn_apply_bwd_keep": (C.c_int, [_vp, _i64, _vp, _i64, _vp, _vp, _vp, _vp, _i32, _f32, _u64, _i32, _vp, _i64, _vp, _i64, _i32,
                                       _vp, _vp, _i32, _i32, _i32, _i32, _i32, _vp, _sz, _vp]),
    "vd_gn_param_sums_batched": (C.c_int, [_vp, _i32, _i64, _vp]),
    "vd_colsum_ws_bytes": (_sz, [_i64, _i32]),
    "vd_colsum": (C.c_int, [_vp, _i64, _i64, _i32, _vp, _i32, _vp, _sz, _vp]),
    "vd_axpby": (C.c_int, [_vp, _i64, _f32, _vp, _i64, _f32, _i64, _i32, _vp]),
    "vd_silu": (C.c_int, [_vp, _vp, _i64, _vp]),
    "vd_silu_bwd": (C.c_int, [_vp, _vp, _vp, _i64, _i32, _vp]),
    "vd_softmax_rows": (C.c_int, [_vp, _i64, _i32, _vp]),
    "vd_softmax_rows_bwd": (C.c_int, [_vp, _vp, _i64, _i32, _f32, _vp]),
    "vd_attn_supported": (C.c_int, [_i32, _i32, _i32]),
    "vd_attn_fwd": (C.c_int, [_vp, _vp, _vp, _i64, _vp, _i64, _vp, _i32, _i32, _i32, _i32, _f32, _vp]),
    "vd_attn_bwd": (C.c_int, [_vp, _vp, _vp, _i64, _vp, _i64, _vp, _i64, _vp, _vp, _vp, _vp, _vp, _i64, _i32, _i32, _i32, _i32, _f32, _vp]),
    "vd_attn_bwd_phase": (C.c_int, [_vp, _vp, _vp, _i64, _vp, _i64, _vp, _i64, _vp, _vp, _vp, _vp, _vp, _i64, _i32, _i32, _i32, _i32, _f32,
                                    _i32, _vp]),
    "vd_nchw_to_nhwc": (C.c_int, [_vp, _vp, _i32, _i32, _i32, _i32, _i64, _vp]),
    "vd_nhwc_to_nchw": (C.c_int, [_vp, _i64, _vp, _i32, _i32, _i32, _i32, _vp]),
    "vd_images_to_uint8_hwc": (C.c_int, [_vp, _vp, _i32, _i32, _i32, _vp]),
    "vd_images_from_uint8_hwc": (C.c_int, [_vp, _vp, _vp, _i32, _i32, _i32, _i32, _vp]),
    "vd_timestep_embedding": (C.c_int, [_vp, _vp, _i32, _i32, _f64, _vp]),
    "vd_class_embed": (C.c_int, [_vp, _vp, _vp, _vp, _i32, _i32, _i32, _vp]),
    "vd_class_embed_bwd": (C.c_int, [_vp, _vp, _vp, _vp, _i32, _i32, _i32, _i32, _vp]),
    "vd_multitag_norm": (C.c_int, [_vp, _vp, _i32, _i32, _vp]),
    "vd_im2col3x3": (C.c_int, [_vp, _i64, _vp, _i32, _i32, _i32, _i32, _vp]),
    "vd_tap_gather": (C.c_int, [_vp, _i64, _vp, _vp, _i64, _i32, _i32, _i32, _i32, _vp]),
    "vd_tap_spread": (C.c_int, [_vp, _i64, _vp, _i64, _i32, _i32, _i32, _i32, _vp]),
    "vd_thin_wgrad_finish": (C.c_int, [_vp, _i32, _i32, _i32, _vp, _i32, _vp, _i32, _i32, _vp, _vp]),
    "vd_q_sample": (C.c_int, [_vp, _vp, _vp, _vp, _i32, _i32, _i32, _vp]),
    "vd_loss_fwd": (C.c_int, [_vp, _vp, _vp, _vp, _vp, _i32, _i32, _vp, _vp, _i32, _i32, _i32, _vp]),
    "vd_loss_bwd": (C.c_int, [_vp, _vp, _vp, _vp, _vp, _vp, _vp, _i32, _i32, _vp, _i32, _i32, _i32, _vp]),
    "vd_bpd_terms": (C.c_int, [_vp, _vp, _vp, _vp, _i32, _i32, _vp, _vp, _vp, _vp, _i32, _i32, _i32, _vp]),
    "vd_bpd_bwd": (C.c_int, [_vp, _vp, _vp, _vp, _vp, _vp, _i32, _i32, _vp, _i32, _i32, _i32, _vp]),
    "vd_sample_step": (C.c_int, [_vp, _vp, _vp, C.POINTER(_f32), _vp, _i32, _i32, _i32, _i32, _vp, _vp, _i32, _i32, _i32, _vp]),
    "vd_bpd_terms_lv": (C.c_int, [_vp, _vp, _vp, _vp, _i32, _i32, _vp, _vp, _vp, _vp, _i32, _i32, _i32, _vp]),
    "vd_bpd_bwd_lv": (C.c_int, [_vp, _vp, _vp, _vp, _vp, _vp, _i32, _i32, _i32, _vp, _i32, _i32, _i32, _vp]),
    "vd_hybrid_loss_fwd": (C.c_int, [_vp, _vp, _vp, _vp, _vp, _vp, _vp, _i32, _i32, _f32, _vp, _vp, _i32, _i32, _i32, _vp]),
    "vd_hybrid_loss_bwd": (C.c_int, [_vp, _vp, _vp, _vp, _vp, _vp, _vp, _vp, _vp, _i32, _i32, _f32, _vp, _i32, _i32, _i32, _vp]),
    "vd_sample_step_lv": (C.c_int, [_vp, _vp, _vp, C.POINTER(_f32), _i32, _i32, _i32, _i32, _vp, _vp, _i32, _i32, _i32, _vp]),
    "vd_distill_mid": (C.c_int, [_vp, _vp, _vp, _i32, _i32, _i32, _vp, _vp, _vp, _vp, _i32, _i32, _i32, _vp]),
    "vd_distill_loss_fwd": (C.c_int, [_vp, _vp, _vp, _vp, _vp, _vp, _vp, _i32, _i32, _i32, _i32, _vp, _vp, _vp, _i32, _i32, _i32, _vp]),
    "vd_distill_loss_bwd": (C.c_int, [_vp, _vp, _vp, _i32, _vp, _i32, _i32, _i32, _vp]),
    "vd_consist_mid": (C.c_int, [_vp, _vp, _vp, _i32, _i32, _i32, _vp, _vp, _vp, _i32, _i32, _i32, _vp]),
    "vd_consist_pair": (C.c_int, [_vp, _vp, _vp, _vp, _vp, _vp, _i32, _i32, _i32, _vp]),
    "vd_consist_loss_fwd": (C.c_int, [_vp, _vp, _vp, _vp, _vp, _vp, _i32, _i32, _f64, _vp, _vp, _vp, _vp, _i32, _i32, _i32, _vp]),
    "vd_consist_loss_bwd": (C.c_int, [_vp, _vp, _vp, _vp, _i32, _vp, _i32, _i32, _i32, _vp]),
    "vd_ema_track_batched": (C.c_int, [_vp, _i32, _i64, _f64, _vp]),
    "vd_solver_step": (C.c_int, [_vp, _vp, _vp, C.POINTER(_f32), _vp, _i32, _i32, _i32, _vp, _vp, _i32, _i32, _i32, _vp]),
    "vd_unipc_step": (C.c_int, [_vp, _vp, _vp, _vp, _vp, C.POINTER(_f32), _vp, _i32, _i32, _i32, _vp, _vp, _vp, _i32, _i32, _i32, _vp]),
    "vd_abs_kth_rows": (C.c_int, [_vp, _i32, _i64, _i64, _vp, _vp]),
    "vd_solver_step_dyn": (C.c_int, [_vp, _vp, _vp, C.POINTER(_f32), _vp, _i32, _i32, _i64, _f32, _vp, _vp, _vp, _i32, _i32, _i32, _vp]),
    "vd_inpaint_step": (C.c_int, [_vp, _vp, _vp, _vp, _vp, _vp, C.POINTER(_f32), _vp, _i32, _i32, _i32, _i32, _i32, _vp, _vp, _i32, _i32, _i32,
                                  _vp]),
    "vd_forward_jump": (C.c_int, [_vp, _vp, C.POINTER(_f32), _vp, _vp, _vp, _i32, _i64, _vp]),
    "vd_noise_extract": (C.c_int, [_vp, _vp, _vp, _vp, C.POINTER(_f32), _vp, _i32, _i32, _i32, _i32, _vp, _vp, _vp, _i32, _i32, _i32, _vp]),
    "vd_slerp_rows": (C.c_int, [_vp, _vp, C.POINTER(_f32), _vp, _vp, _vp, _i32, _i64, _vp]),
    "vd_lsm_draw": (C.c_int, [_vp, _vp, _vp, _vp, _vp, _vp, _vp, _i32, _i32, _i32, _f64, _vp]),
    "vd_lsm_update": (C.c_int, [_vp, _vp, _vp, _vp, _vp, _i32, _i32, _i32, _vp]),
    "vd_sumsq_ws_bytes": (_sz, [_i64]),
    "vd_sumsq": (C.c_int, [_vp, _i64, _vp, _vp, _sz, _vp]),
    "vd_adamw_ema": (C.c_int, [_vp, _vp, _vp, _vp, _vp, _i64, _vp, _f32, _f32, _f32, _f32, _f32, _f32, _f32, _f32, _f32, _i64, _i64, _i32,
                               _f32, _f32, _vp]),
    "vd_adamw_ema_flagged": (C.c_int, [_vp, _vp, _vp, _vp, _vp, _i64, _vp, _f32, _f32, _f32, _f32, _f32, _f32, _f32, _f32, _f32, _i64, _i64,
                                       _vp, _vp, _f64, _f64, _vp]),
    "vd_rows_sqnorm_f16": (C.c_int, [_vp, _i64, _i32, _vp, _vp]),
    "vd_knn_kth_ws_bytes": (_sz, [_i64, _i64, _i32]),
    "vd_knn_kth_f16": (C.c_int, [_vp, _vp, _i64, _vp, _vp, _i64, _i32, _i32, _vp, _vp, _sz, _vp]),
    "vd_manifold_hits_ws_bytes": (_sz, [_i64]),
# ... 217 lines not shown
    with _TimedName("wino_conv_kernel<{tw}, {ns}, {st}, false, 0>", 2.0 * nimg * H * W * Cout * 9 * Cin) as t:
        _check(lib().vd_conv3x3_wino(ptr(x), ldx, ptr(U), ptr(bias), ptr(res), ldres, ptr(y), ldy, nimg, H, W, Cin, Cout,
                                     ptr(stats_part), stream()), "vd_conv3x3_wino")
        if PROFILE is not None:
            k = lib().vd_wino_last_kernel()
            if k < 0:
                k = -k
                t.name = f"wino_conv_wide_kernel<{k // 2000}, {(k // 2) % 1000}, {'true' if k & 1 else 'false'}>"
            else:
                t.name = t.name.format(tw=k // 2000, ns=(k // 2) % 1000, st="true" if k & 1 else "false")
            _note_bytes(t.name, 4.0 * (nimg * H * W * (Cin + Cout + (Cout if res is not None else 0)) + 16 * Cout * Cin))


def mfma_calibrate(seconds=1.5, blocks=256, iters=20000):
    import time
    sink = torch.zeros(1, device="cuda")
    stamps = torch.zeros(2 * blocks, dtype=torch.int64, device="cuda")
    e0, e1 = torch.cuda.Event(enable_timing=True), torch.cuda.Event(enable_timing=True)
    t_end = time.perf_counter() + seconds
    ms = 0.0
    while True:
        e0.record()
        _check(lib().vd_mfma_calibrate(sink.data_ptr(), stamps.data_ptr(), blocks, iters, 12345, stream()), "vd_mfma_calibrate")
        e1.record()
        torch.cuda.synchronize()
        ms = e0.elapsed_time(e1)
        if time.perf_counter() >= t_end:
            break
    st = stamps.view(blocks, 2).double().cpu()
    mhz = float((st[:, 0] / st[:, 1].clamp(min=1)).median()) * 100.0
    tflops = blocks * 8 * iters * 16 * 2048.0 / (ms * 1e-3) / 1e12
    return mhz, tflops


WINO43 = os.environ.get("VD_WINO43", "1") != "0"
WINO43_MIN_W = int(os.environ.get("VD_WINO43_MIN_W", "16"))


WINO43_OCC = os.environ.get("VD_WINO43_OCC", "1") != "0"


def wino43_preferred(nimg, H, W, N):
    return not WINO43_OCC or bool(lib().vd_conv3x3_wino43_preferred(nimg, H, W, N))


def wino43_supported(nimg, H, W, Cin, Cout, lddy, lddx):
    return (WINO and WINO43 and W >= WINO43_MIN_W and bool(lib().vd_conv3x3_dgrad_wino43_supported(nimg, H, W, Cin, Cout, lddy, lddx))
            and wino43_preferred(nimg, H, W, Cin))


def wino43_pack(w, Cout, Cin, U43):
    _check(lib().vd_wino43_pack(ptr(w), Cout, Cin, ptr(U43), stream()), "vd_wino43_pack")


def wino43_pack_batched(table, n, total_blocks):
    assert table.is_cuda and table.dtype == torch.int64 and table.is_contiguous()
    _check(lib().vd_wino43_pack_batched(table.data_ptr(), n, total_blocks, stream()), "vd_wino43_pack_batched")


WINO43_FWD = os.environ.get("VD_WINO43_FWD", "1") != "0"


def wino43_fwd_supported(nimg, H, W, Cin, Cout, ldx, ldy, ldres=0):
    return (WINO and WINO43_FWD and bool(lib().vd_conv3x3_wino43_fwd_supported(nimg, H, W, Cin, Cout, ldx, ldy, ldres))
            and wino43_preferred(nimg, H, W, Cout))


def wino43_pack_fwd(w, Cout, Cin, U43f):
    _check(lib().vd_wino43_pack_fwd(ptr(w), Cout, Cin, ptr(U43f), stream()), "vd_wino43_pack_fwd")


def wino43_fwd_chunk_rows(H, W):
    return int(lib().vd_conv3x3_wino43_fwd_chunk_rows(H, W))


def conv3x3_wino43_fwd(x, ldx, U43f, bias, y, ldy, nimg, H, W, Cin, Cout, res=None, ldres=0, stats_part=None):
    name = f"wino43_conv_kernel<{W // 4}, true>"
    with _TimedName(name, 2.0 * nimg * H * W * Cout * 9 * Cin):
        _check(lib().vd_conv3x3_wino43_fwd(ptr(x), ldx, ptr(U43f), ptr(bias), ptr(res), ldres, ptr(y), ldy, nimg, H, W, Cin, Cout,
                                           ptr(stats_part), stream()), "vd_conv3x3_wino43_fwd")
    _note_bytes(name, 4.0 * (nimg * H * W * (Cin + Cout + (Cout if res is not None else 0)) + 36 * Cout * Cin))


def conv3x3_dgrad_wino43(dy, lddy, U43, dx, lddx, nimg, H, W, Cin, Cout):
    with _TimedName(f"wino43_conv_kernel<{W // 4}, false>", 2.0 * nimg * H * W * Cout * 9 * Cin):
        _check(lib().vd_conv3x3_dgrad_wino43(ptr(dy), lddy, ptr(U43), ptr(dx), lddx, nimg, H, W, Cin, Cout, stream()),
               "vd_conv3x3_dgrad_wino43")
    _note_bytes(f"wino43_conv_kernel<{W // 4}, false>", 4.0 * (nimg * H * W * (Cin + Cout) + 36 * Cout * Cin))


def conv3x3(x, ldx, wpack, bias, y, ldy, nimg, H, W, Cin, Cout, res=None, ldres=0, accumulate=False, stats_part=None):
    with _TimedTile("gemm_dma_kernel<{tile}, 2, 0, false, {kt}>", 2.0 * nimg * H * W * Cout * 9 * Cin):
        _check(lib().vd_conv3x3(ptr(x), ldx, ptr(wpack), ptr(bias), ptr(res), ldres, ptr(y), ldy, nimg, H, W, Cin, Cout,
                                int(accumulate), ptr(stats_part), stream()), "vd_conv3x3")


def conv3x3_wgrad_wino(x, ldx, dy, lddy, nimg, H, W, Cin, Cout, dw, Cin_w, Cout_w, accumulate=False, dbias=None):
    nb = lib().vd_conv3x3_wgrad_wino_ws_bytes(nimg, H, W, Cin, Cout)
    ws = workspace(nb, x.device, "wgrad")
    args = _wgrad_args(x, ldx, dy, lddy, nimg, H, W, Cin, Cout, dw, dbias, Cin_w, Cout_w, accumulate, ws)
    if PROFILE is None:
        _check(lib().vd_conv3x3_wgrad_wino(*args, stream()), "vd_conv3x3_wgrad_wino")
        return
    tws = min(W // 2, 16)
    with _TimedName(f"wino_wgrad_kernel<{tws}, {'true' if dbias is not None else 'false'}>", 2.0 * nimg * H * W * Cout * 9 * Cin):
        _check(lib().vd_conv3x3_wgrad_wino_phase(*args, 1, stream()), "vd_conv3x3_wgrad_wino_phase")
    with _TimedName("wino_wgrad_reduce_kernel", 0.0):
        _check(lib().vd_conv3x3_wgrad_wino_phase(*args, 2, stream()), "vd_conv3x3_wgrad_wino_phase")


WGRAD_STREAM = os.environ.get("VD_WGRAD_STREAM", "1") != "0"
GROUPED_AUTO_SPLIT = os.environ.get("VD_GROUPED_AUTO_SPLIT", "1") != "0"
GN_FOLD = os.environ.get("VD_GN_FOLD", "1") != "0"
GN_FOLD_MAX_CHUNKS = int(os.environ.get("VD_GN_FOLD_MAX_CHUNKS", "8"))
READY_PER_BLOCK = os.environ.get("VD_READY_PER_BLOCK", "0") != "0"
AUTOGRAD_CHAIN = os.environ.get("VD_AUTOGRAD_CHAIN", "1") != "0"
WINO43_WGRAD = os.environ.get("VD_WINO43_WGRAD", "1") != "0"
WINO43_WGRAD_MIN_TILES = int(os.environ.get("VD_WINO43_WGRAD_MIN_TILES", "512"))


W43_WGRAD_TAG = "[36 planes of the F(4x4,3x3) weight gradient]"


def wgrad43_supported(nimg, H, W, Cin, Cout, ldx, lddy):
    return (WINO and WINO43_WGRAD and nimg * (H // 4) * (W // 4) >= WINO43_WGRAD_MIN_TILES
            and bool(lib().vd_conv3x3_wgrad_wino43_supported(nimg, H, W, Cin, Cout, ldx, lddy)))


def conv3x3_wgrad_wino43(x, ldx, dy, lddy, nimg, H, W, Cin, Cout, dw, Cin_w, Cout_w, accumulate=False, dbias=None):
    nb = lib().vd_conv3x3_wgrad_wino43_ws_bytes(nimg, H, W, Cin, Cout)
    ws = workspace(nb, x.device, "wgrad43")
    args = _wgrad_args(x, ldx, dy, lddy, nimg, H, W, Cin, Cout, dw, dbias, Cin_w, Cout_w, accumulate, ws)
    if PROFILE is None:
        _check(lib().vd_conv3x3_wgrad_wino43(*args, stream()), "vd_conv3x3_wgrad_wino43")
        return
    with _TimedBytes("wino43_wgrad_transform_kernel", 4.0 * nimg * H * W * (Cin + Cout) * (1 + 2.25)):
        _check(lib().vd_conv3x3_wgrad_wino43_phase(*args, 1, stream()), "vd_conv3x3_wgrad_wino43_phase")
    with _TimedTile("gemm_dma_kernel<{tile}, 1, 1, true, {kt}, true> " + W43_WGRAD_TAG, 2.0 * nimg * H * W * Cout * 9 * Cin) as t:
        _check(lib().vd_conv3x3_wgrad_wino43_phase(*args, 2, stream()), "vd_conv3x3_wgrad_wino43_phase")
    _note_bytes(PROFILE[-1][0], 4.0 * (36.0 * nimg * (H // 4) * (W // 4) * (Cin + Cout) + 36.0 * Cout * Cin))
    with _TimedName("wino43_wgrad_finish_kernel", 0.0):
        _check(lib().vd_conv3x3_wgrad_wino43_phase(*args, 4, stream()), "vd_conv3x3_wgrad_wino43_phase")


def conv3x3_wgrad(x, ldx, dy, lddy, nimg, H, W, Cin, Cout, dw, Cin_w, Cout_w, accumulate=False, dbias=None, direct=False):
    if not direct and wgrad43_supported(nimg, H, W, Cin, Cout, ldx, lddy):
        return conv3x3_wgrad_wino43(x, ldx, dy, lddy, nimg, H, W, Cin, Cout, dw, Cin_w, Cout_w, accumulate, dbias)
    if WINO and not direct and lib().vd_conv3x3_wgrad_wino_supported(nimg, H, W, Cin, Cout, ldx, lddy):
        return conv3x3_wgrad_wino(x, ldx, dy, lddy, nimg, H, W, Cin, Cout, dw, Cin_w, Cout_w, accumulate, dbias)
    nb = lib().vd_conv3x3_wgrad_ws_bytes(nimg, H, W, Cin, Cout)
    ws = workspace(nb, x.device, "wgrad")
    args = _wgrad_args(x, ldx, dy, lddy, nimg, H, W, Cin, Cout, dw, dbias, Cin_w, Cout_w, accumulate, ws)
    flops = 2.0 * nimg * H * W * Cout * 9 * Cin
    if PROFILE is None:
        _check(lib().vd_conv3x3_wgrad(*args, stream()), "vd_conv3x3_wgrad")
        return
    with _TimedTile("gemm_dma_kernel<{tile}, 1, 2, true, {kt}>", flops):
        _check(lib().vd_conv3x3_wgrad_phase(*args, 1, stream()), "vd_conv3x3_wgrad_phase")
    with _TimedTile("reduce_slabs_oihw_kernel", 0.0):
        _check(lib().vd_conv3x3_wgrad_phase(*args, 2, stream()), "vd_conv3x3_wgrad_phase")


def im2col3x3(x, ldx, xc, nimg, H, W, Cc):
    _check(lib().vd_im2col3x3(ptr(x), ldx, ptr(xc), nimg, H, W, Cc, stream()), "vd_im2col3x3")


def tap_gather(z, ldz, bias, out, ldo, nimg, H, W, Cout):
    _check(lib().vd_tap_gather(ptr(z), ldz, ptr(bias), ptr(out), ldo, nimg, H, W, Cout, stream()), "vd_tap_gather")


def tap_spread(dy, lddy, dz, ldz, nimg, H, W, Cout):
    _check(lib().vd_tap_spread(ptr(dy), lddy, ptr(dz), ldz, nimg, H, W, Cout, stream()), "vd_tap_spread")


def thin_wgrad_finish(g, Cout_w, Cin, Cin_w, dw, accumulate=False, colsum=None, cs_stride=1, cs_off=0, dbias=None):
    _check(lib().vd_thin_wgrad_finish(ptr(g), Cout_w, Cin, Cin_w, ptr(dw), int(accumulate), ptr(colsum), cs_stride, cs_off,
                                      ptr(dbias), stream()), "vd_thin_wgrad_finish")


def pack_conv3x3(w, Cout_w, Cin_w, wf=None, Cin_p=0, wd=None, Cout_p=0):
    _check(lib().vd_pack_conv3x3(ptr(w), Cout_w, Cin_w, ptr(wf), Cin_p, ptr(wd), Cout_p, stream()), "vd_pack_conv3x3")


def pack_conv3x3_batched(table, n, total_blocks):
    assert table.is_cuda and table.dtype == torch.int64 and table.is_contiguous()
    _check(lib().vd_pack_conv3x3_batched(table.data_ptr(), n, total_blocks, stream()), "vd_pack_conv3x3_batched")


def gn_stats(x, ldx, nimg, HW, Cc, stats, G=32, eps=1e-6):
    nb = lib().vd_gn_ws_bytes(nimg, HW, Cc)
    ws = workspace(nb, x.device, "gn")
    _check(lib().vd_gn_stats(ptr(x), ldx, nimg, HW, Cc, G, eps, ptr(stats), ws.data_ptr(), ws.numel() * 4, stream()),
           "vd_gn_stats")


def _gn_bwd_name():
    k = lib().vd_gn_bwd_last_kernel()
    if k > 0:
        split, k = k // 100000000, k % 100000000
        nt, k = k >= 1000000, k % 1000000
        return f"gn_bwd_fused_kernel<{k // 10000}, {k % 10000}, {'true' if nt else 'false'}, {'true' if split else 'false'}>"
    return "gn_bwd_apply_kernel (two-pass form)" if k < 0 else "gn_bwd_apply_kernel (resample)"


def gn_apply(x, ldx, stats, gamma, beta, film, act, p_drop, seed, resample, y, ldy, nimg, H, W, Cc, coef, G=32):
    with _TimedBytes("gn_apply_kernel" if gamma is not None else "gn_apply_kernel (resample)", 4.0 * nimg * Cc * (H * W + _resampled_hw(H, W, resample))):
        _gn_apply(x, ldx, stats, gamma, beta, film, act, p_drop, seed, resample, y, ldy, nimg, H, W, Cc, coef, G)


def gn_apply_from_partials(x, ldx, parts, gamma, beta, film, act, p_drop, seed, resample, y, ldy, nimg, H, W, Cc, coef, G=32, eps=1e-6):
    with _TimedBytes("gn_apply_kernel", 4.0 * nimg * Cc * (H * W + _resampled_hw(H, W, resample))):
        _check(lib().vd_gn_apply_from_partials(ptr(x), ldx, *_two_parts(parts), ptr(gamma), ptr(beta), ptr(film), int(act),
                                               float(p_drop), int(seed), resample, ptr(y), ldy, nimg, H, W, Cc, G, eps, ptr(coef), stream()),
               "vd_gn_apply_from_partials")


def _gn_apply(x, ldx, stats, gamma, beta, film, act, p_drop, seed, resample, y, ldy, nimg, H, W, Cc, coef, G=32):
    _check(lib().vd_gn_apply(ptr(x), ldx, ptr(stats), ptr(gamma), ptr(beta), ptr(film), int(act), float(p_drop), int(seed),
                             resample, ptr(y), ldy, nimg, H, W, Cc, G, ptr(coef), stream()), "vd_gn_apply")


def gn_apply_bwd(dy, lddy, x, ldx, coef, gamma, beta, film, act, p_drop, seed, resample, add, ldadd, dx, lddx,
                 accumulate_dx, dfilm, dgamma, dbeta, accumulate_params, nimg, H, W, Cc, G=32, pgb_keep=None):
    nb = lib().vd_gn_ws_bytes(nimg, H * W, Cc)
    ws = workspace(nb, dy.device, "gn")
    nbytes = 4.0 * nimg * Cc * (_resampled_hw(H, W, resample) + H * W * (1 + (gamma is not None) + (add is not None) + bool(accumulate_dx)))
    with _TimedBytes("gn_apply_bwd", nbytes, rename=_gn_bwd_name):
        if pgb_keep is not None:
# ... 420 lines not shown
```

### v-diffusion-torch_amd/v_diffusion/engine.py

```python
import collections
import contextlib
import math

import torch

from . import _hip as H

GROUPS = 32
EPS = 1e-6
THIN = 8


def _ld(t):
    return t.stride(2)


def _chk(t):
    B, Hh, Ww, C = t.shape
    ld = t.stride(2)
    assert t.stride(3) == 1 and t.stride(1) == Ww * ld and t.stride(0) == Hh * Ww * ld, "not an NHWC view"
    return B, Hh, Ww, C, ld


def _splitk(M, N, K, n=1):
# ... 145 lines not shown
                getattr(H, launch)(*self.tables[name])

    def image(self, w, dgrad):
        co, ci = w.shape[0], w.shape[1]
        U = self.fallback.get((id(w), dgrad))
        if U is None:
            U = self.fallback[(id(w), dgrad)] = torch.empty((16, ci, co) if dgrad else (16, co, ci), dtype=torch.float32, device=w.device)
        H.wino_pack(w, co, ci, **{"ud" if dgrad else "uf": U})
        return U


class _Cat:
    __slots__ = ("buf", "parts")

    def __init__(self, buf):
        self.buf, self.parts = buf, {}

    def joined(self, ch_h):
        pa, pb = self.parts.get(0), self.parts.get(ch_h)
        return pa + pb if (pa is not None and pb is not None) else None


class UNetEngine:

    def __init__(self, model):
        self.m = model
        self.levels = len(model.ch_multipliers)
        self.plan, self.pushes, self.film_groups = _plan(model)
        self.film_slot = {b.res_prefix: b.film for b in self.plan if b.res is not None}
        self._pack_lru = {}
        self._packs = None
        self._fixed = None
        self._norm_channels = sum(p.numel() for k, p in model.named_parameters()
                                  if k.endswith(".weight") and p.ndim == 1)
        self._pgb_arena = self._pgb_table = None
        self._side = self._side_stream = None
        self._wq = None
        self._active_run = None
        self._segments = None

    @staticmethod
    def _new(ref, *shape):
        return torch.empty(shape, dtype=torch.float32, device=ref.device)

    def _res_of(self, level, H0, W0):
        return H0 >> level, W0 >> level

    def _part(self, ref, nimg, HW, C):
        if HW % 32:
            return None
        return torch.empty(H.stats_part_numel(nimg, HW, C), dtype=torch.float32, device=ref.device)

    @staticmethod
    def _parts(part, C, HW, rows=None):
        if part is None:
            return None
        return [(part, C, HW // (rows or (H.last_row_tile() // 2)))]

    def _norm(self, x, x_parts, gn, film, act, p_drop, seed, rs, y, B, Hh, Ww, C):
        coef = self._new(x, B, 4, C)
        stats = None
        if x_parts is not None and H.GN_FOLD and max(k for _, _, k in x_parts) <= H.GN_FOLD_MAX_CHUNKS:
            H.gn_apply_from_partials(x, _ld(x), x_parts, gn.weight, gn.bias, film, act, p_drop, seed, rs, y, _ld(y), B, Hh, Ww, C, coef,
                                     GROUPS, EPS)
            return coef
        if x_parts is not None:
            H.gn_coef_from_partials(x_parts, B, Hh * Ww, gn.weight, gn.bias, film, coef, GROUPS, EPS)
        else:
            stats = self._new(x, B, GROUPS, 2)
            H.gn_stats(x, _ld(x), B, Hh * Ww, C, stats, GROUPS, EPS)
        H.gn_apply(x, _ld(x), stats, gn.weight, gn.bias, film, act, p_drop, seed, rs, y, _ld(y), B, Hh, Ww, C, coef, GROUPS)
        return coef

    def _wgrad(self, dy, x, dw, db, M, N, K, lda, ldb, ldc):
        if self._wq is None or not H.GROUPED_WGRAD:
            H.gemm(dy, x, dw, M, N, K, a_kind=H.COL, b_kind=H.COL, lda=lda, ldb=ldb, ldc=ldc, splitk=_splitk(M, N, K), colsum=db)
            return
        key = (M, N, K, lda, ldb, ldc, db is not None)
        q = self._wq.setdefault(key, [])
        q.append((dy, x, dw, db))
        if len(q) == H.GROUP_MAX:
            self._wgrad_flush_key(key)

    def _cwgrad(self, x, ldx, dy, lddy, *args, **kw):
        side = self._side
        if side is None:
            return H.conv3x3_wgrad(x, ldx, dy, lddy, *args, **kw)
        side.wait_stream(torch.cuda.current_stream())
        x.record_stream(side)
        dy.record_stream(side)
        with torch.cuda.stream(side):
            H.conv3x3_wgrad(x, ldx, dy, lddy, *args, **kw)

    def _side_join(self):
        if self._side is not None:
            torch.cuda.current_stream().wait_stream(self._side)

    def _wgrad_flush_key(self, key):
        q = self._wq.pop(key, None)
        if not q:
            return
        M, N, K, lda, ldb, ldc, _ = key
        ok = M % 4 == 0 and N % 4 == 0 and lda % 4 == 0 and ldb % 4 == 0 and max(lda, ldb, ldc) * 128 + 128 < 0x70000000 // 4 and \
            all(dy.data_ptr() % 16 == 0 and x.data_ptr() % 16 == 0 for dy, x, _, _ in q)
        if len(q) == 1 or not ok:
            for dy, x, dw, db in q:
                H.gemm(dy, x, dw, M, N, K, a_kind=H.COL, b_kind=H.COL, lda=lda, ldb=ldb, ldc=ldc, splitk=_splitk(M, N, K), colsum=db)
            return
        S = H.lib().vd_gemm_grouped_wgrad_auto_split(len(q), M, N, K, 1, 64) if H.GROUPED_AUTO_SPLIT else _splitk(M, N, K, len(q))
        H.gemm_grouped_wgrad(q, M, N, K, lda, ldb, ldc, S)

    def _wgrad_flush(self):
        if not self._wq:
            return
        side = self._side
        if side is None:
            for key in list(self._wq):
                self._wgrad_flush_key(key)
            return
        side.wait_stream(torch.cuda.current_stream())
        for q in self._wq.values():
            for dy, x, _, _ in q:
                dy.record_stream(side)
                x.record_stream(side)
        with torch.cuda.stream(side):
            for key in list(self._wq):
                self._wgrad_flush_key(key)

    def _pgb_begin(self, ref, B):
        need = B * 2 * self._norm_channels
        if self._pgb_arena is None or self._pgb_arena.numel() < need or self._pgb_arena.device != ref.device:
            self._pgb_arena = torch.empty(need, dtype=torch.float32, device=ref.device)
            self._pgb_table = None
        self._pgb_rows, self._pgb_off, self._pgb_blk = [], 0, 0

    def _pgb(self, B, C, dgamma, dbeta):
        sl = self._pgb_arena[self._pgb_off: self._pgb_off + B * 2 * C]
        self._pgb_rows.append([sl.data_ptr(), dgamma.data_ptr(), dbeta.data_ptr(), B, C, 0, 0, self._pgb_blk])
        self._pgb_off += B * 2 * C
        self._pgb_blk += (C + 15) // 16
        return sl

    def _pgb_finish(self):
        key = tuple(tuple(r) for r in self._pgb_rows)
        if self._pgb_table is None or self._pgb_table[0] != key:
            self._pgb_table = (key, torch.tensor(self._pgb_rows, dtype=torch.int64).to(self._pgb_arena.device))
        H.gn_param_sums_batched(self._pgb_table[1], len(self._pgb_rows), self._pgb_blk)

    PACK_STATES_MAX = 4

    def _conv_geoms(self, B, H0, W0):
        out = []
        for b in self.plan:
            if b.res is None:
                continue
            lh, lw = H._resampled(*self._res_of(b.level, H0, W0), b.rs)
            out.append((b.res.conv1.weight, B, lh, lw, b.cin, b.cout))
            out.append((b.res.conv2.weight, B, lh, lw, b.cout, b.cout))
        return out

    def _pack_all(self, need_d, geom=None):
        ws = [c.weight for b in self.plan if b.res is not None for c in (b.res.conv1, b.res.conv2)]
        key = (bool(need_d), H.WINO, H.WINO43_FWD, geom) + tuple(w.data_ptr() for w in ws)
        pk = self._pack_lru.pop(key, None)
        if pk is None:
            pk = ConvPacks(ws, need_d, self._conv_geoms(*geom) if geom is not None else [])
            while len(self._pack_lru) >= self.PACK_STATES_MAX:
                self._pack_lru.pop(next(iter(self._pack_lru)))
        self._pack_lru[key] = self._packs = pk
        pk.repack()
        return pk

    @property
    def packs(self):
        return self._packs

    @contextlib.contextmanager
    def fixed_weights(self):
        self._fixed = {}
        try:
            yield
        finally:
            self._fixed = None

    def _layer(self, w):
        return self._packs.layers.get(id(w), _NO_PACK) if self._packs is not None else _NO_PACK

    def _conv(self, x, ldx, w, bias, y, ldy, B, Hh, Ww, Cin, Cout, dgrad=False, res=None, ldres=0, stats_part=None):
        pk, p = self._packs, self._layer(w)
        if not dgrad and p.u43f is not None and H.wino43_fwd_supported(B, Hh, Ww, Cin, Cout, ldx, ldy, ldres if res is not None else 0):
            H.conv3x3_wino43_fwd(x, ldx, p.u43f, bias, y, ldy, B, Hh, Ww, Cin, Cout, res=res, ldres=ldres, stats_part=stats_part)
            return H.wino43_fwd_chunk_rows(Hh, Ww)
        if dgrad and p.u43 is not None and H.wino43_supported(B, Hh, Ww, Cout, Cin, ldx, ldy):
            assert res is None and bias is None and stats_part is None
            H.conv3x3_dgrad_wino43(x, ldx, p.u43, y, ldy, B, Hh, Ww, Cout, Cin)
            return None
        if p is not _NO_PACK and pk.wino and H.wino_supported(B, Hh, Ww, Cin, Cout, ldx, ldy, ldres if res is not None else 0):
            U = p.ud if dgrad else p.uf
            if U is None:
                U = pk.image(w, dgrad)
            H.conv3x3_wino(x, ldx, U, bias, y, ldy, B, Hh, Ww, Cin, Cout, res=res, ldres=ldres, stats_part=stats_part)
            return H.last_row_tile() // 2
        H.conv3x3(x, ldx, self._pack_d(w) if dgrad else self._pack_f(w), bias, y, ldy, B, Hh, Ww, Cin, Cout, res=res, ldres=ldres,
                  stats_part=stats_part)
        return H.last_row_tile() // 2

    def _pack_f(self, w, cin_p=None):
        p = self._layer(w)
        if p.wf is not None:
            return p.wf
        cache = self._fixed
        if cache is not None and id(w) in cache:
            return cache[id(w)]
        co, ci = w.shape[0], w.shape[1]
        cin_p = cin_p or ci
        wf = self._new(w, co, 9, cin_p)
        H.pack_conv3x3(w, co, ci, wf=wf, Cin_p=cin_p)
        if cache is not None:
            cache[id(w)] = wf
        return wf

    def _pack_d(self, w, cout_p=None):
        p = self._layer(w)
        if p.wd is not None:
            return p.wd
        co, ci = w.shape[0], w.shape[1]
        cout_p = cout_p or co
        wd = self._new(w, ci, 9, cout_p)
        H.pack_conv3x3(w, co, ci, wd=wd, Cout_p=cout_p)
        return wd

    def _pack_thin(self, w, rows):
        cache = self._fixed
        key = ("thin", id(w))
        if cache is not None and key in cache:
            return cache[key]
        co, ci = w.shape[0], w.shape[1]
        wz = torch.zeros((rows, ci), dtype=torch.float32, device=w.device)
        H.pack_conv3x3(w, co, ci, wf=wz, Cin_p=ci)
        if cache is not None:
            cache[key] = wz
        return wz

    @staticmethod
    def _linear(x, w, b, out, accumulate=False):
        M, K = x.shape
        N = w.shape[0]
        H.gemm(x, w, out, M, N, K, a_kind=H.ROW, b_kind=H.ROW, lda=x.stride(0), ldb=w.stride(0), ldc=out.stride(0), bias=b,
               accumulate=accumulate)

    def _linear_bwd(self, x, w, dy, dw, db, dx, dx_accumulate=False):
        M, K = x.shape
        N = w.shape[0]
        self._wgrad(dy, x, dw, db, N, K, M, dy.stride(0), x.stride(0), K)
        if dx is not None:
            H.gemm(dy, w, dx, M, K, N, a_kind=H.ROW, b_kind=H.COL, lda=dy.stride(0), ldb=w.stride(0), ldc=dx.stride(0),
                   accumulate=dx_accumulate)

    def _embed_fwd(self, t, y, tape):
        m = self.m
        B = t.shape[0]
        dev_ref = m.in_conv.weight
        if t.dtype != torch.float64:
            t = t.to(torch.float64)
        te0 = self._new(dev_ref, B, m.hid_channels)
        H.timestep_embedding(t.contiguous(), te0, B, m.hid_channels)
        l0, l2 = m.time_embed[0], m.time_embed[2]
        h0 = self._new(dev_ref, B, m.embedding_dim)
        self._linear(te0, l0.weight, l0.bias, h0)
        a0 = torch.empty_like(h0)
        H.silu(h0, a0)
        te = torch.empty_like(h0)
        self._linear(a0, l2.weight, l2.bias, te)
        yn = None
        if m.num_classes and y is not None:
            y = y.to(torch.float32).contiguous().clone()
            if m.multitags:
                assert y.ndim == 2 and y.shape[1] == m.num_classes
                yn = torch.empty_like(y)
                H.multitag_norm(y, yn, B, m.num_classes)
                self._linear(yn, m.class_embed.weight, m.class_embed.bias, te, accumulate=True)
            else:
                lin = m.class_embed[1]
                H.class_embed(y.reshape(-1), lin.weight, lin.bias, te, B, m.embedding_dim, m.num_classes)
                yn = y.reshape(-1)
        ta = torch.empty_like(te)
        H.silu(te, ta)
        if tape is not None:
            tape["embed"] = dict(te0=te0, h0=h0, a0=a0, te=te, yn=yn)
        return ta

    def _embed_bwd(self, ctx, dta, G):
        m = self.m
        B = dta.shape[0]
        te0, h0, a0, te, yn = ctx["te0"], ctx["h0"], ctx["a0"], ctx["te"], ctx["yn"]
        dte = torch.empty_like(dta)
        H.silu_bwd(te, dta, dte)
        if yn is not None:
            if m.multitags:
                self._linear_bwd(yn, m.class_embed.weight, dte, G["class_embed.weight"], G["class_embed.bias"], None)
            else:
                H.class_embed_bwd(yn, dte, G["class_embed.1.weight"], G["class_embed.1.bias"], B, m.embedding_dim, m.num_classes)
        elif m.num_classes:
            for k in G:
                if k.startswith("class_embed."):
                    G[k].zero_()
        l0, l2 = m.time_embed[0], m.time_embed[2]
        da0 = torch.empty_like(dte)
        self._linear_bwd(a0, l2.weight, dte, G["time_embed.2.weight"], G["time_embed.2.bias"], da0)
        dh0 = torch.empty_like(da0)
        H.silu_bwd(h0, da0, dh0)
        self._linear_bwd(te0, l0.weight, dh0, G["time_embed.0.weight"], G["time_embed.0.bias"], None)

    def _film_fwd(self, ta, tape):
        B, E = ta.shape
        films, stacks = {}, {}
        cache = self._fixed
        for c2, mods in self.film_groups.items():
            key = ("film", c2)
            if cache is not None and key in cache:
                W, bv = cache[key]
            else:
                W = torch.stack([mm.fc.weight.detach() for mm in mods])
                bv = torch.stack([mm.fc.bias.detach() for mm in mods])
                if cache is not None:
                    cache[key] = (W, bv)
            nb = len(mods)
            out = self._new(ta, nb, B, c2)
            H.gemm(ta, W, out, B, c2, E, a_kind=H.ROW, b_kind=H.ROW, lda=E, ldb=E, ldc=c2, bias=bv, sBias=c2, batch=nb,
                   sA=(0, 0), sB=(c2 * E, 0), sC=(B * c2, 0))
            films[c2], stacks[c2] = out, W
        if tape is not None:
            tape["film_w"] = stacks
        return films

    def _film_bwd(self, dfilms, stacks, dta):
        B, E = dta.shape
        for c2, df in dfilms.items():
            nb, W = df.shape[0], stacks[c2]
            P = self._new(dta, nb, B * E)
            H.gemm(df, W, P, B, E, c2, a_kind=H.ROW, b_kind=H.COL, lda=c2, ldb=E, ldc=E, batch=nb, sA=(B * c2, 0), sB=(c2 * E, 0),
                   sC=(B * E, 0))
            H.colsum(P, B * E, nb, B * E, dta.view(-1), accumulate=True)

    def _res_fwd(self, blk, x, films, dest, p_drop, seed, tape, x_parts=None):
        mod, prefix = blk.res, blk.res_prefix
        B, Hh, Ww, Cin, ldx = _chk(x)
        Cout, rs = blk.cout, blk.rs
        Ho, Wo = H._resampled(Hh, Ww, rs)
        a1 = self._new(x, B, Ho, Wo, Cin)
        coef1 = self._norm(x, x_parts, mod.norm1, None, 1, 0.0, 0, rs, a1, B, Hh, Ww, Cin)
        h1 = self._new(x, B, Ho, Wo, Cout)
        ph = self._part(x, B, Ho * Wo, Cout)
        rows = self._conv(a1, Cin, mod.conv1.weight, mod.conv1.bias, h1, Cout, B, Ho, Wo, Cin, Cout, stats_part=ph)
        h1_parts = self._parts(ph, Cout, Ho * Wo, rows)
        c2, fi = blk.film
        film = films[c2][fi]
        a2 = self._new(x, B, Ho, Wo, Cout)
        coef2 = self._norm(h1, h1_parts, mod.norm2, film, 1, p_drop, seed, H.RS_NONE, a2, B, Ho, Wo, Cout)
        if rs != H.RS_NONE:
            xs = self._new(x, B, Ho, Wo, Cin)
            H.gn_apply(x, ldx, None, None, None, None, 0, 0.0, 0, rs, xs, Cin, B, Hh, Ww, Cin, None, GROUPS)
        else:
            xs = x
        has_skip = Cin != Cout
        if has_skip:
            sk = self._new(x, B, Ho, Wo, Cout)
            w = mod.skip.weight
            H.gemm(xs, w, sk, B * Ho * Wo, Cout, Cin, a_kind=H.ROW, b_kind=H.ROW, lda=_ld(xs), ldb=Cin, ldc=Cout, bias=mod.skip.bias)
        else:
            sk = xs
        pd = self._part(x, B, Ho * Wo, Cout)
        rows = self._conv(a2, Cout, mod.conv2.weight, mod.conv2.bias, dest, _ld(dest), B, Ho, Wo, Cout, Cout, res=sk,
                          ldres=_ld(sk), stats_part=pd)
        out_parts = self._parts(pd, Cout, Ho * Wo, rows)
        if tape is not None:
            tape[prefix] = dict(x=x, coef1=coef1, a1=a1, h1=h1, coef2=coef2, a2=a2, film=film, xs=xs if has_skip else None,
                                seed=seed, p=p_drop)
        return out_parts

    def _res_bwd(self, blk, ctx, dy, dx, dx_accumulate, ta, dfilms, G):
        mod = blk.res
        g = {s: G[name] for s, name in blk.res_names.items()}
        x, a1, h1, a2, film = ctx["x"], ctx["a1"], ctx["h1"], ctx["a2"], ctx["film"]
        B, Hh, Ww, Cin, ldx = _chk(x)
        _, Ho, Wo, Cout, lddy = _chk(dy)
        rs = blk.rs
        self._cwgrad(a2, Cout, dy, lddy, B, Ho, Wo, Cout, Cout, g["conv2.weight"], Cout, Cout, dbias=g["conv2.bias"])
        da2 = self._new(x, B, Ho, Wo, Cout)
        self._conv(dy, lddy, mod.conv2.weight, None, da2, Cout, B, Ho, Wo, Cout, Cout, dgrad=True)
        dh1 = self._new(x, B, Ho, Wo, Cout)
        c2, fi = blk.film
        dfilm = dfilms[c2][fi]
        H.gn_apply_bwd(da2, Cout, h1, Cout, ctx["coef2"], mod.norm2.weight, mod.norm2.bias, film, 1, ctx["p"], ctx["seed"],
                       H.RS_NONE, None, 0, dh1, Cout, False, dfilm, None, None, False, B, Ho, Wo, Cout, GROUPS,
                       pgb_keep=self._pgb(B, Cout, g["norm2.weight"], g["norm2.bias"]))
        del da2
        self._cwgrad(a1, Cin, dh1, Cout, B, Ho, Wo, Cin, Cout, g["conv1.weight"], Cin, Cout, dbias=g["conv1.bias"])
        da1 = self._new(x, B, Ho, Wo, Cin)
        self._conv(dh1, Cout, mod.conv1.weight, None, da1, Cin, B, Ho, Wo, Cout, Cin, dgrad=True)
        del dh1
        if Cin != Cout:
            xs = ctx["xs"]
            P = B * Ho * Wo
            w = mod.skip.weight
            self._wgrad(dy, xs, g["skip.weight"], g["skip.bias"], Cout, Cin, P, lddy, _ld(xs), Cin)
            dsk = self._new(x, B, Ho, Wo, Cin)
            H.gemm(dy, w, dsk, P, Cin, Cout, a_kind=H.ROW, b_kind=H.COL, lda=lddy, ldb=Cin, ldc=Cin)
        else:
            dsk = dy
        if rs != H.RS_NONE:
            addt = self._new(x, B, Hh, Ww, Cin)
            H.gn_apply_bwd(dsk, _ld(dsk), None, 0, None, None, None, None, 0, 0.0, 0, rs, None, 0, addt, Cin, False, None, None,
                           None, False, B, Hh, Ww, Cin, GROUPS)
        else:
            addt = dsk
        H.gn_apply_bwd(da1, Cin, x, ldx, ctx["coef1"], mod.norm1.weight, mod.norm1.bias, None, 1, 0.0, 0, rs, addt, _ld(addt),
                       dx, _ld(dx), dx_accumulate, None, None, None, False, B, Hh, Ww, Cin, GROUPS,
                       pgb_keep=self._pgb(B, Cin, g["norm1.weight"], g["norm1.bias"]))
        self._linear_bwd(ta, mod.fc.weight, dfilm, g["fc.weight"], g["fc.bias"], None)

    def _attn_fwd(self, blk, x, dest, tape, x_parts=None):
        mod, prefix = blk.att, blk.att_prefix
        B, Hh, Ww, C, ldx = _chk(x)
        L, nh, hd = Hh * Ww, mod.num_heads, mod.head_dim
        hid = nh * hd
        xn = self._new(x, B, Hh, Ww, C)
        coef = self._norm(x, x_parts, mod.norm, None, 0, 0.0, 0, H.RS_NONE, xn, B, Hh, Ww, C)
        qkv = self._new(x, B, L, 3 * hid)
        H.gemm(xn, mod.proj_in.weight, qkv, B * L, 3 * hid, C, a_kind=H.ROW, b_kind=H.ROW, lda=C, ldb=C, ldc=3 * hid,
               bias=mod.proj_in.bias)
        ld = 3 * hid
        alpha = 1.0 / math.sqrt(hd)
        q, k, v = qkv[0, 0, 0:], qkv[0, 0, hid:], qkv[0, 0, 2 * hid:]
        O = self._new(x, B, L, hid)
        S = lse = None
        if B * nh <= 65535 and H.attn_use_fused(L, hd, B * nh, tape is not None):
            if tape is not None:
                lse = self._new(x, B * nh * L)
            H.attn_fwd(q, k, v, ld, O, hid, lse, B, nh, L, hd, alpha)
        else:
            S = self._new(x, B, nh, L, L)
            H.gemm(q, k, S, L, L, hd, a_kind=H.ROW, b_kind=H.ROW, lda=ld, ldb=ld, ldc=L, batch=B * nh, nh=nh, sA=(L * ld, hd),
                   sB=(L * ld, hd), sC=(nh * L * L, L * L), alpha=alpha)
            H.softmax_rows(S, B * nh * L, L)
            H.gemm(S, v, O, L, hd, L, a_kind=H.ROW, b_kind=H.COL, lda=L, ldb=ld, ldc=hid, batch=B * nh, nh=nh, sA=(nh * L * L, L * L),
                   sB=(L * ld, hd), sC=(L * hid, hd))
        pd = self._part(x, B, L, C)
        if pd is not None and L % 64:
            pd = None
        H.gemm(O, mod.proj_out.weight, dest, B * L, C, hid, a_kind=H.ROW, b_kind=H.ROW, lda=hid, ldb=hid, ldc=_ld(dest),
               bias=mod.proj_out.bias, R=x, ldr=ldx, stats=pd, stats_hw=L)
        out_parts = self._parts(pd, C, L)
        if tape is not None:
            tape[prefix] = dict(x=x, coef=coef, xn=xn, qkv=qkv, P=S, O=O, lse=lse)
        return out_parts

    def _attn_bwd(self, blk, ctx, dy, dx, dx_accumulate, G):
        mod = blk.att
        g = {s: G[name] for s, name in blk.att_names.items()}
        x, xn, qkv, P, O = ctx["x"], ctx["xn"], ctx["qkv"], ctx["P"], ctx["O"]
        B, Hh, Ww, C, ldx = _chk(x)
        lddy = _ld(dy)
        L, nh, hd = Hh * Ww, mod.num_heads, mod.head_dim
        hid, ld = nh * hd, 3 * nh * hd
        M = B * L
        self._wgrad(dy, O, g["proj_out.weight"], g["proj_out.bias"], C, hid, M, lddy, hid, hid)
        dO = self._new(x, B, L, hid)
        H.gemm(dy, mod.proj_out.weight, dO, M, hid, C, a_kind=H.ROW, b_kind=H.COL, lda=lddy, ldb=hid, ldc=hid)
        dqkv = self._new(x, B, L, ld)
        q, k, v = qkv[0, 0, 0:], qkv[0, 0, hid:], qkv[0, 0, 2 * hid:]
        dq, dk, dv = dqkv[0, 0, 0:], dqkv[0, 0, hid:], dqkv[0, 0, 2 * hid:]
        sP, sQ, sO = (nh * L * L, L * L), (L * ld, hd), (L * hid, hd)
        alpha = 1.0 / math.sqrt(hd)
        if P is None:
            H.attn_bwd(q, k, v, ld, O, hid, dO, hid, ctx["lse"], self._new(x, B * nh * L), dq, dk, dv, ld, B, nh, L, hd, alpha)
        else:
            H.gemm(P, dO, dv, L, hd, L, a_kind=H.COL, b_kind=H.COL, lda=L, ldb=hid, ldc=ld, batch=B * nh, nh=nh, sA=sP, sB=sO, sC=sQ)
            dP = self._new(x, B, nh, L, L)
            H.gemm(dO, v, dP, L, L, hd, a_kind=H.ROW, b_kind=H.ROW, lda=hid, ldb=ld, ldc=L, batch=B * nh, nh=nh, sA=sO, sB=sQ, sC=sP)
            H.softmax_rows_bwd(P, dP, B * nh * L, L, alpha)
# ... 261 lines not shown
```

Baseline: 2185.

## Add plane-layout Winograd F(4x4,3x3) forward that keeps V for weight gradient

Adds a three-phase Winograd forward for large-tile training convs: the input transform writes V planes, a row-blocked GEMM multiplies them by weight planes packed on the fly, and a new output-transform kernel applies bias, residual and group-norm stats. The transformed input V is kept on the tape, so the backward weight-gradient pass skips recomputing the input transform and the activation tensors a1/a2 are no longer stored. This costs a large V buffer (36 planes per tile times Cin) and extra GEMM workspace per conv, which raises memory traffic and footprint in exchange for less backward work.

Result: faster. 2277, median of 6 (+4.2%).

```diff
diff --git a/include/vdiff_hip.h b/include/vdiff_hip.h
--- a/include/vdiff_hip.h
+++ b/include/vdiff_hip.h
@@ -100,6 +100,18 @@
                                   int32_t Cin, int32_t Cout, float* dw_oihw, float* dbias, int32_t Cin_w, int32_t Cout_w,
                                   int32_t accumulate, float* ws, size_t ws_bytes, int32_t phase, void* stream);
 int vd_wino43_wgrad_last_kernel(void);
+
+int vd_conv3x3_wino43_fwd_planes_supported(int32_t nimg, int32_t H, int32_t W, int32_t Cin, int32_t Cout, int64_t ldx, int64_t ldy,
+                                           int64_t ldres);
+size_t vd_conv3x3_wino43_v_floats(int32_t nimg, int32_t H, int32_t W, int32_t Cin);
+size_t vd_conv3x3_wino43_fwd_planes_ws_bytes(int32_t nimg, int32_t H, int32_t W, int32_t Cin, int32_t Cout);
+int vd_conv3x3_fwd_planes_preferred(int32_t nimg, int32_t H, int32_t W, int32_t Cin, int32_t Cout, int32_t training);
+int vd_conv3x3_wino43_fwd_planes(const float* xin, int64_t ldx, const float* w_oihw, const float* bias, const float* res, int64_t ldres,
+                                 float* y, int64_t ldy, int32_t nimg, int32_t H, int32_t W, int32_t Cin, int32_t Cout, float* stats_part,
+                                 float* V, float* ws, size_t ws_bytes, int32_t phase, void* stream);
+int vd_conv3x3_wgrad_wino43_v(const float* V, const float* dy, int64_t lddy, int32_t nimg, int32_t H, int32_t W, int32_t Cin, int32_t Cout,
+                              float* dw_oihw, float* dbias, int32_t Cin_w, int32_t Cout_w, int32_t accumulate, float* ws, size_t ws_bytes,
+                              int32_t phase, void* stream);
 
 int vd_wino_pack_batched(const int64_t* items_dev, int32_t n, int64_t total_blocks, void* stream);
 
diff --git a/v-diffusion-torch_amd/csrc/common.h b/v-diffusion-torch_amd/csrc/common.h
--- a/v-diffusion-torch_amd/csrc/common.h
+++ b/v-diffusion-torch_amd/csrc/common.h
@@ -22,6 +22,7 @@
                                int32_t N, int32_t K, int64_t lda, int64_t ldb, int64_t ldc, int32_t splitk, float* ws, size_t ws_bytes,
                                void* stream, int64_t a_kblk, int64_t b_kblk, int32_t slabs_only);
 int vd_gemm_grouped_wgrad_used_slabs(int32_t count, int32_t M, int32_t N, int32_t K, int32_t splitk);
+int vd_gemm_rowblk(const vd_gemm_desc* d, int64_t a_rblk, void* stream);
 extern thread_local int vd_g_last_tile;
 inline int vd_tile_code(bool tr, bool spl, int kt, int bm, int bn) {
     return ((((tr ? 1 : 0) + (spl ? 2 : 0)) * 100 + kt) * 1000 + bm) * 1000 + bn;
diff --git a/v-diffusion-torch_amd/csrc/gemm.hip b/v-diffusion-torch_amd/csrc/gemm.hip
--- a/v-diffusion-torch_amd/csrc/gemm.hip
+++ b/v-diffusion-torch_amd/csrc/gemm.hip
@@ -449,7 +449,8 @@
             const int c = (lane % RLPR) ^ swz_of<KT>(row);
             const int m = m0 + row;
             kcA[j] = c * 4;
-            voA[j] = (m < p.M) ? (unsigned)(row * (int)p.lda + c * 4) * 4u : OOB;
+            const int rowoff = (!GROUPED && AK == VD_ROW && p.a_kblk) ? (row >> 4) * (int)p.a_kblk + (row & 15) * (int)p.lda : row * (int)p.lda;
+            voA[j] = (m < p.M) ? (unsigned)(rowoff + c * 4) * 4u : OOB;
             unsigned mk = 0;
             if (AK == VD_IM2COL) {
                 int y, x;
@@ -479,7 +480,7 @@
             else by[j] = bx[j] = 0;
         }
     }
-    const float* Ablk = (AK == VD_COL) ? A + m0 : A + (long long)m0 * p.lda;
+    const float* Ablk = (AK == VD_COL) ? A + m0 : ((!GROUPED && AK == VD_ROW && p.a_kblk) ? A + (long long)(m0 >> 4) * p.a_kblk : A + (long long)m0 * p.lda);
     const float* Bblk = (BK == VD_ROW) ? B + (long long)n0 * p.ldb : ((BK == VD_COL) ? B + n0 : B + ci0);
     const long long tapoffB = (BK == VD_IM2COL) ? (long long)((tapN / 3 - 1) * p.W + (tapN % 3 - 1)) * p.ldb : 0;
 
@@ -1320,7 +1321,7 @@
     else launch_tile2<AK, BK, false>(P, a, grid, st);
 }
 
-int run_gemm(const vd_gemm_desc& d, hipStream_t st) {
+int run_gemm(const vd_gemm_desc& d, hipStream_t st, long long a_rblk = 0) {
     VD_REQUIRE(d.M > 0 && d.N > 0 && d.K > 0, "vd_gemm: empty problem M=%d N=%d K=%d", d.M, d.N, d.K);
     VD_REQUIRE(d.A && d.B && d.C, "vd_gemm: null operand");
     VD_REQUIRE(vd_aligned16(d.A) && vd_aligned16(d.B), "vd_gemm: A/B must be 16-byte aligned");
@@ -1351,6 +1352,11 @@
     a.colsum = d.colsum; a.colsum_accumulate = d.colsum_accumulate;
     a.stats = d.stats; a.stats_hw = d.stats_hw;
     a.sBias = d.sBias;
+    a.group_S = 0; a.a_kblk = a_rblk; a.b_kblk = 0;
+    if (a_rblk) {
+        VD_REQUIRE(ak == VD_ROW && bk == VD_ROW && d.splitk <= 1 && d.M % 16 == 0 && a_rblk > 0 && a_rblk % 4 == 0 && use_dma(a) &&
+                   16 * a_rblk + 16 * d.lda + 256 < 0x70000000LL / 4, "vd_gemm_rowblk: needs ROW/ROW operands, M %% 16 == 0 and a block pitch in range");
+    }
     a.lgW = a.lgHW = -1;
     if ((conv || wgrad) && (d.W & (d.W - 1)) == 0 && ((d.H * d.W) & (d.H * d.W - 1)) == 0) {
         a.lgW = __builtin_ctz((unsigned)d.W); a.lgHW = __builtin_ctz((unsigned)(d.H * d.W));
@@ -1569,6 +1575,11 @@
     return run_gemm(*d, (hipStream_t)stream);
 }
 
+int vd_gemm_rowblk(const vd_gemm_desc* d, int64_t a_rblk, void* stream) {
+    VD_REQUIRE(d != nullptr, "vd_gemm_rowblk: null descriptor");
+    return run_gemm(*d, (hipStream_t)stream, a_rblk);
+}
+
 extern "C" int vd_conv3x3(const float* xin, int64_t ldx, const float* wpack, const float* bias, const float* res,
                           int64_t ldres, float* y, int64_t ldy, int32_t nimg, int32_t H, int32_t W, int32_t Cin,
                           int32_t Cout, int32_t accumulate, float* stats_part, void* stream) {
diff --git a/v-diffusion-torch_amd/csrc/wino43.hip b/v-diffusion-torch_amd/csrc/wino43.hip
--- a/v-diffusion-torch_amd/csrc/wino43.hip
+++ b/v-diffusion-torch_amd/csrc/wino43.hip
@@ -1,4 +1,5 @@
 #include "common.h"
+#include <stdlib.h>
 #include <type_traits>
 
 namespace {
@@ -514,6 +515,7 @@
     const float* x; long long ldx; const float* dy; long long lddy;
     float* V; float* dM;
     int nimg, H, W, Cin, Cout, TW, TPI, T;
+    int z0;
 };
 
 __global__ __launch_bounds__(256) void wino43_wgrad_transform_kernel(const WgT43 p) {
@@ -522,7 +524,7 @@
     const int img = tile / p.TPI, tin = tile - img * p.TPI;
     const int ty = tin / p.TW, tx = tin - ty * p.TW;
     const int c4 = 4 * quad;
-    if (blockIdx.z == 0) {
+    if ((int)blockIdx.z + p.z0 == 0) {
         if (c4 >= p.Cin) return;
         f32x4 R[6][6];
 #pragma unroll
@@ -668,6 +670,99 @@
     o[0] = accumulate ? o[0] + w0 : w0;
     o[1] = accumulate ? o[1] + w1 : w1;
     o[2] = accumulate ? o[2] + w2 : w2;
+}
+
+__global__ __launch_bounds__(256) void wino43_pack_planes_kernel(const float* w, float* U, int Cout, int Cin) {
+    const long long idx = (long long)blockIdx.x * 256 + threadIdx.x, plane = (long long)Cout * Cin;
+    if (idx >= plane) return;
+    const float* src = w + idx * 9;
+    const double Gd[6][3] = {{64.0 / 81, 0.0, 0.0}, {-128.0 / 243, -32.0 / 81, -8.0 / 27}, {-128.0 / 243, 32.0 / 81, -8.0 / 27},
+                             {32.0 / 243, 16.0 / 81, 8.0 / 27}, {32.0 / 243, -16.0 / 81, 8.0 / 27}, {0.0, 0.0, 1.0}};
+    double g[3][3], tmp[6][3];
+#pragma unroll
+    for (int a = 0; a < 3; ++a)
+#pragma unroll
+        for (int b = 0; b < 3; ++b) g[a][b] = (double)src[a * 3 + b];
+#pragma unroll
+    for (int a = 0; a < 6; ++a)
+#pragma unroll
+        for (int c = 0; c < 3; ++c) tmp[a][c] = Gd[a][0] * g[0][c] + Gd[a][1] * g[1][c] + Gd[a][2] * g[2][c];
+#pragma unroll
+    for (int a = 0; a < 6; ++a)
+#pragma unroll
+        for (int b = 0; b < 6; ++b) U[(6 * a + b) * plane + idx] = (float)(tmp[a][0] * Gd[b][0] + tmp[a][1] * Gd[b][1] + tmp[a][2] * Gd[b][2]);
+}
+
+__device__ __forceinline__ void at4(const f32x4 (&m)[6], f32x4 (&o)[4]) {
+    const f32x4 p12 = m[1] + m[2], q12 = m[1] - m[2], p34 = m[3] + m[4], q34 = m[3] - m[4];
+    o[0] = m[0] + p12 + p34;
+    o[1] = 0.75f * q12 + 1.5f * q34;
+    o[2] = 0.5625f * p12 + 2.25f * p34;
+    o[3] = 0.421875f * q12 + 3.375f * q34 + m[5];
+}
+
+struct Out43 {
+    const float* M; long long plane;
+    const float* bias; const float* res; long long ldr;
+    float* y; long long ldy;
+    float* stats;
+    int H, W, Cout, TW, TPI, T, CT;
+};
+
+__global__ __launch_bounds__(256) void wino43_out_transform_kernel(const Out43 p) {
+    __shared__ float ssum[2][16][64];
+    const int q = threadIdx.x, tl = threadIdx.y;
+    const int c4 = blockIdx.y * 64 + 4 * q;
+    const bool in = c4 < p.Cout;
+    f32x4 s1 = {0.f, 0.f, 0.f, 0.f}, s2 = s1;
+    if (in) {
+        f32x4 bv = {0.f, 0.f, 0.f, 0.f};
+        if (p.bias) bv = *reinterpret_cast<const f32x4*>(p.bias + c4);
+        for (int i = 0; i < p.CT; i += 16) {
+            const int tile = blockIdx.x * p.CT + i + tl;
+            if (tile >= p.T) break;
+            const int img = tile / p.TPI, tin = tile - img * p.TPI;
+            const int ty = tin / p.TW, tx = tin - ty * p.TW;
+            const float* mp = p.M + (long long)tile * p.Cout + c4;
+            f32x4 S[6][4];
+#pragma unroll
+            for (int a = 0; a < 6; ++a) {
+                f32x4 m[6];
+#pragma unroll
+                for (int b = 0; b < 6; ++b) m[b] = *reinterpret_cast<const f32x4*>(mp + (long long)(6 * a + b) * p.plane);
+                at4(m, S[a]);
+            }
+            const long long pix0 = ((long long)img * p.H + 4 * ty) * p.W + 4 * tx;
+#pragma unroll
+            for (int v = 0; v < 4; ++v) {
+                const f32x4 col[6] = {S[0][v], S[1][v], S[2][v], S[3][v], S[4][v], S[5][v]};
+                f32x4 o[4];
+                at4(col, o);
+#pragma unroll
+                for (int u = 0; u < 4; ++u) {
+                    const long long pix = pix0 + (long long)u * p.W + v;
+                    f32x4 val = o[u] + bv;
+                    if (p.res) val += *reinterpret_cast<const f32x4*>(p.res + pix * p.ldr + c4);
+                    s1 += val; s2 += val * val;
+                    *reinterpret_cast<f32x4*>(p.y + pix * p.ldy + c4) = val;
+                }
+            }
+        }
+    }
+    if (!p.stats) return;
+#pragma unroll
+    for (int j = 0; j < 4; ++j) { ssum[0][tl][4 * q + j] = s1[j]; ssum[1][tl][4 * q + j] = s2[j]; }
+    __syncthreads();
+    const int tid = tl * 16 + q;
+    if (tid < 128) {
+        const int st = tid >> 6, ch = tid & 63;
+        if (blockIdx.y * 64 + ch < p.Cout) {
+            float v = 0.f;
+#pragma unroll
+            for (int k = 0; k < 16; ++k) v += ssum[st][k][ch];
+            p.stats[((long long)blockIdx.x * 2 + st) * p.Cout + blockIdx.y * 64 + ch] = v;
+        }
+    }
 }
 
 struct Wg43Plan { bool ok; int T, S; size_t v_f, m_f, u_f, cs_f, gemm_bytes; };
@@ -683,6 +778,15 @@
     return g;
 }
 
+#ifndef VD_PLANES_MIN_TILES
+#define VD_PLANES_MIN_TILES 8192
+#endif
+#ifndef VD_PLANES_TRAINING
+#define VD_PLANES_TRAINING 1
+#endif
+#ifndef VD_PLANES_INFERENCE
+#define VD_PLANES_INFERENCE 0
+#endif
 thread_local int g_last43 = 0;
 #ifdef VD_PROBES
 unsigned long long* g_probe43 = nullptr;
@@ -825,26 +929,28 @@
 
 static int wgrad43_impl(const float* xin, int64_t ldx, const float* dy, int64_t lddy, int32_t nimg, int32_t H, int32_t W, int32_t Cin,
                         int32_t Cout, float* dw_oihw, float* dbias, int32_t Cin_w, int32_t Cout_w, int32_t accumulate, float* ws,
-                        size_t ws_bytes, void* stream, int phases) {
-    VD_REQUIRE(xin && dy && dw_oihw && ws, "vd_conv3x3_wgrad_wino43: null operand");
+                        size_t ws_bytes, void* stream, int phases, const float* Vgiven = nullptr) {
+    VD_REQUIRE((xin || Vgiven) && dy && dw_oihw && ws, "vd_conv3x3_wgrad_wino43: null operand");
+    VD_REQUIRE(!Vgiven || vd_aligned16(Vgiven), "vd_conv3x3_wgrad_wino43: V must be 16-byte aligned");
     VD_REQUIRE(vd_conv3x3_wgrad_wino43_supported(nimg, H, W, Cin, Cout, ldx, lddy),
                "vd_conv3x3_wgrad_wino43: unsupported geometry nimg=%d H=%d W=%d Cin=%d Cout=%d", nimg, H, W, Cin, Cout);
     VD_REQUIRE(Cin_w <= Cin && Cout_w <= Cout, "vd_conv3x3_wgrad_wino43: real dims exceed padded dims");
-    VD_REQUIRE(vd_aligned16(xin) && vd_aligned16(dy) && vd_aligned16(ws), "vd_conv3x3_wgrad_wino43: operands must be 16-byte aligned");
+    VD_REQUIRE((!xin || vd_aligned16(xin)) && vd_aligned16(dy) && vd_aligned16(ws), "vd_conv3x3_wgrad_wino43: operands must be 16-byte aligned");
     VD_REQUIRE(ws_bytes >= vd_conv3x3_wgrad_wino43_ws_bytes(nimg, H, W, Cin, Cout), "vd_conv3x3_wgrad_wino43: workspace too small");
     const Wg43Plan g = wg43_plan(nimg, H, W, Cin, Cout);
-    float* V = ws;
-    float* dM = V + g.v_f;
+    const float* V = Vgiven ? Vgiven : ws;
+    float* dM = ws + g.v_f;
     float* dU = dM + g.m_f;
     float* cs = dU + g.u_f;
     float* gws = cs + g.cs_f;
     hipStream_t st = (hipStream_t)stream;
     if (phases & 1) {
         WgT43 t = {};
-        t.x = xin; t.ldx = ldx; t.dy = dy; t.lddy = lddy; t.V = V; t.dM = dM;
+        t.x = xin; t.ldx = ldx; t.dy = dy; t.lddy = lddy; t.V = ws; t.dM = dM;
         t.nimg = nimg; t.H = H; t.W = W; t.Cin = Cin; t.Cout = Cout; t.TW = W / 4; t.TPI = (H / 4) * (W / 4); t.T = g.T;
-        const int cmax = Cin > Cout ? Cin : Cout;
-        hipLaunchKernelGGL(wino43_wgrad_transform_kernel, dim3((unsigned)(g.T / 4), (unsigned)((cmax + 255) / 256), 2), dim3(64, 4), 0, st, t);
+        t.z0 = Vgiven ? 1 : 0;
+        const int cmax = Vgiven ? Cout : (Cin > Cout ? Cin : Cout);
+        hipLaunchKernelGGL(wino43_wgrad_transform_kernel, dim3((unsigned)(g.T / 4), (unsigned)((cmax + 255) / 256), Vgiven ? 1 : 2), dim3(64, 4), 0, st, t);
         VD_LAUNCH_CHECK("wino43_wgrad_transform_kernel");
     }
     if (phases & 2) {
@@ -888,3 +994,85 @@
 }
 
 extern "C" int vd_wino43_wgrad_last_kernel(void) { return g_last43w; }
+
+extern "C" int vd_conv3x3_wgrad_wino43_v(const float* V, const float* dy, int64_t lddy, int32_t nimg, int32_t H, int32_t W, int32_t Cin,
+                                         int32_t Cout, float* dw_oihw, float* dbias, int32_t Cin_w, int32_t Cout_w, int32_t accumulate,
+                                         float* ws, size_t ws_bytes, int32_t phase, void* stream) {
+    VD_REQUIRE(V, "vd_conv3x3_wgrad_wino43_v: null V");
+    VD_REQUIRE(phase == 7 || phase == 1 || phase == 2 || phase == 4, "vd_conv3x3_wgrad_wino43_v: phase must be 7, 1, 2 or 4");
+    return wgrad43_impl(nullptr, Cin, dy, lddy, nimg, H, W, Cin, Cout, dw_oihw, dbias, Cin_w, Cout_w, accumulate, ws, ws_bytes, stream, phase, V);
+}
+
+extern "C" int vd_conv3x3_wino43_fwd_planes_supported(int32_t nimg, int32_t H, int32_t W, int32_t Cin, int32_t Cout, int64_t ldx, int64_t ldy,
+                                                      int64_t ldres) {
+    if (nimg <= 0 || Cin <= 0 || Cout <= 0 || Cin % 4 || Cout % 4 || ldx % 4 || ldy % 4 || ldres % 4) return 0;
+    if (!((W == 32 && H == 32) || (W == 64 && H % 16 == 0 && H >= 16) || (W == 16 && H == 16))) return 0;
+    const long long T = (long long)nimg * (H / 4) * (W / 4);
+    if (T >= (1LL << 22) || 36LL * 16 * Cin * 16 + 16LL * Cin + 256 >= 0x70000000LL / 4) return 0;
+    if (128LL * Cin + 128 >= 0x70000000LL / 4 || 128LL * Cout + 128 >= 0x70000000LL / 4) return 0;
+    return 1;
+}
+
+extern "C" size_t vd_conv3x3_wino43_v_floats(int32_t nimg, int32_t H, int32_t W, int32_t Cin) {
+    return (size_t)36 * ((size_t)nimg * (H / 4) * (W / 4)) * Cin;
+}
+
+extern "C" size_t vd_conv3x3_wino43_fwd_planes_ws_bytes(int32_t nimg, int32_t H, int32_t W, int32_t Cin, int32_t Cout) {
+    const size_t T = (size_t)nimg * (H / 4) * (W / 4);
+    return ((size_t)36 * Cout * Cin + (size_t)36 * T * Cout) * sizeof(float);
+}
+
+extern "C" int vd_conv3x3_fwd_planes_preferred(int32_t nimg, int32_t H, int32_t W, int32_t Cin, int32_t Cout, int32_t training) {
+    if (!vd_conv3x3_wino43_fwd_planes_supported(nimg, H, W, Cin, Cout, Cin, Cout, Cout)) return 0;
+    const long long T = (long long)nimg * (H / 4) * (W / 4);
+    static const long long floor_t = getenv("VD_PLANES_MIN_TILES") ? atoll(getenv("VD_PLANES_MIN_TILES")) : VD_PLANES_MIN_TILES;
+    static const int inference = getenv("VD_PLANES_INFERENCE") ? atoi(getenv("VD_PLANES_INFERENCE")) : VD_PLANES_INFERENCE;
+    if (T < floor_t || Cout % 256 || Cin % 16) return 0;
+    return training ? VD_PLANES_TRAINING : (inference != 0);
+}
+
+extern "C" int vd_conv3x3_wino43_fwd_planes(const float* xin, int64_t ldx, const float* w_oihw, const float* bias, const float* res,
+                                            int64_t ldres, float* y, int64_t ldy, int32_t nimg, int32_t H, int32_t W, int32_t Cin,
+                                            int32_t Cout, float* stats_part, float* V, float* ws, size_t ws_bytes, int32_t phase, void* stream) {
+    VD_REQUIRE(xin && w_oihw && y && V && ws, "vd_conv3x3_wino43_fwd_planes: null operand");
+    VD_REQUIRE(vd_conv3x3_wino43_fwd_planes_supported(nimg, H, W, Cin, Cout, ldx, ldy, res ? ldres : 0),
+               "vd_conv3x3_wino43_fwd_planes: unsupported geometry nimg=%d H=%d W=%d Cin=%d Cout=%d", nimg, H, W, Cin, Cout);
+    VD_REQUIRE(vd_aligned16(xin) && vd_aligned16(y) && vd_aligned16(V) && vd_aligned16(ws) && (!res || vd_aligned16(res)) &&
+               (!bias || vd_aligned16(bias)), "vd_conv3x3_wino43_fwd_planes: operands must be 16-byte aligned");
+    VD_REQUIRE(ws_bytes >= vd_conv3x3_wino43_fwd_planes_ws_bytes(nimg, H, W, Cin, Cout), "vd_conv3x3_wino43_fwd_planes: workspace too small");
+    VD_REQUIRE(phase == 7 || phase == 1 || phase == 2 || phase == 4, "vd_conv3x3_wino43_fwd_planes: phase must be 7, 1, 2 or 4");
+    const int TPI = (H / 4) * (W / 4), T = nimg * TPI;
+    float* Up = ws;
+    float* Mb = ws + (size_t)36 * Cout * Cin;
+    hipStream_t st = (hipStream_t)stream;
+    if (phase & 1) {
+        const long long plane = (long long)Cout * Cin;
+        hipLaunchKernelGGL(wino43_pack_planes_kernel, dim3((unsigned)((plane + 255) / 256)), dim3(256), 0, st, w_oihw, Up, Cout, Cin);
+        VD_LAUNCH_CHECK("wino43_pack_planes_kernel");
+        WgT43 t = {};
+        t.x = xin; t.ldx = ldx; t.V = V;
+        t.nimg = nimg; t.H = H; t.W = W; t.Cin = Cin; t.Cout = Cout; t.TW = W / 4; t.TPI = TPI; t.T = T;
+        t.z0 = 0;
+        hipLaunchKernelGGL(wino43_wgrad_transform_kernel, dim3((unsigned)(T / 4), (unsigned)((Cin + 255) / 256), 1), dim3(64, 4), 0, st, t);
+        VD_LAUNCH_CHECK("wino43_wgrad_transform_kernel(V)");
+    }
+    if (phase & 2) {
+        vd_gemm_desc d = {};
+        d.A = V; d.B = Up; d.C = Mb;
+        d.M = T; d.N = Cout; d.K = Cin; d.a_kind = VD_ROW; d.b_kind = VD_ROW;
+        d.lda = Cin; d.ldb = Cin; d.ldc = Cout;
+        d.batch = 36; d.nh = 1; d.alpha = 1.f;
+        d.sAb = 16LL * Cin; d.sBb = (long long)Cout * Cin; d.sCb = (long long)T * Cout;
+        const int rc = vd_gemm_rowblk(&d, 36LL * 16 * Cin, stream);
+        if (rc) return rc;
+    }
+    if (phase & 4) {
+        Out43 o = {};
+        o.M = Mb; o.plane = (long long)T * Cout; o.bias = bias; o.res = res; o.ldr = ldres; o.y = y; o.ldy = ldy; o.stats = stats_part;
+        o.H = H; o.W = W; o.Cout = Cout; o.TW = W / 4; o.TPI = TPI; o.T = T;
+        o.CT = vd_conv3x3_wino43_fwd_chunk_rows(H, W) / 16;
+        hipLaunchKernelGGL(wino43_out_transform_kernel, dim3((unsigned)(T / o.CT), (unsigned)((Cout + 63) / 64)), dim3(16, 16), 0, st, o);
+        VD_LAUNCH_CHECK("wino43_out_transform_kernel");
+    }
+    return 0;
+}
diff --git a/v-diffusion-torch_amd/v_diffusion/_hip.py b/v-diffusion-torch_amd/v_diffusion/_hip.py
--- a/v-diffusion-torch_amd/v_diffusion/_hip.py
+++ b/v-diffusion-torch_amd/v_diffusion/_hip.py
@@ -67,6 +67,13 @@
     "vd_conv3x3_wgrad_wino43_ws_bytes": (_sz, [_i32, _i32, _i32, _i32, _i32]),
     "vd_conv3x3_wgrad_wino43": (C.c_int, [_vp, _i64, _vp, _i64, _i32, _i32, _i32, _i32, _i32, _vp, _vp, _i32, _i32, _i32, _vp, _sz, _vp]),
     "vd_wino43_wgrad_last_kernel": (C.c_int, []),
+    "vd_conv3x3_wino43_fwd_planes_supported": (C.c_int, [_i32, _i32, _i32, _i32, _i32, _i64, _i64, _i64]),
+    "vd_conv3x3_wino43_v_floats": (_sz, [_i32, _i32, _i32, _i32]),
+    "vd_conv3x3_wino43_fwd_planes_ws_bytes": (_sz, [_i32, _i32, _i32, _i32, _i32]),
+    "vd_conv3x3_fwd_planes_preferred": (C.c_int, [_i32, _i32, _i32, _i32, _i32, _i32]),
+    "vd_conv3x3_wino43_fwd_planes": (C.c_int, [_vp, _i64, _vp, _vp, _vp, _i64, _vp, _i64, _i32, _i32, _i32, _i32, _i32, _vp, _vp, _vp, _sz,
+                                               _i32, _vp]),
+    "vd_conv3x3_wgrad_wino43_v": (C.c_int, [_vp, _vp, _i64, _i32, _i32, _i32, _i32, _i32, _vp, _vp, _i32, _i32, _i32, _vp, _sz, _i32, _vp]),
     "vd_conv3x3_wgrad_wino43_phase": (C.c_int, [_vp, _i64, _vp, _i64, _i32, _i32, _i32, _i32, _i32, _vp, _vp, _i32, _i32, _i32, _vp, _sz, _i32, _vp]),
     "vd_gn_stats_from_partials": (C.c_int, [_vp, _i32, _i32, _vp, _i32, _i32, _i32, _i32, _i32, _f32, _vp, _vp]),
     "vd_gn_coef_from_partials": (C.c_int, [_vp, _i32, _i32, _vp, _i32, _i32, _i32, _i32, _i32, _f32, _vp, _vp, _vp, _vp, _vp]),
@@ -450,6 +457,45 @@
     _note_bytes(name, 4.0 * (nimg * H * W * (Cin + Cout + (Cout if res is not None else 0)) + 36 * Cout * Cin))
 
 
+CONV_PLANES = os.environ.get("VD_CONV_PLANES", "1")
+
+
+def conv3x3_fwd_planes_preferred(nimg, H, W, Cin, Cout, training):
+    return bool(lib().vd_conv3x3_fwd_planes_preferred(nimg, H, W, Cin, Cout, int(bool(training))))
+
+
+def conv_planes_supported(nimg, H, W, Cin, Cout, ldx, ldy, ldres=0, training=False):
+    if CONV_PLANES == "0" or not (WINO and WINO43_FWD):
+        return False
+    if not lib().vd_conv3x3_wino43_fwd_planes_supported(nimg, H, W, Cin, Cout, ldx, ldy, ldres):
+        return False
+    if training and not wgrad43_supported(nimg, H, W, Cin, Cout, Cin, Cout):
+        return False
+    return CONV_PLANES == "2" or conv3x3_fwd_planes_preferred(nimg, H, W, Cin, Cout, training)
+
+
+def conv3x3_wino43_fwd_planes(x, ldx, w, bias, y, ldy, nimg, H, W, Cin, Cout, res=None, ldres=0, stats_part=None, v=None):
+    nv = lib().vd_conv3x3_wino43_v_floats(nimg, H, W, Cin)
+    if v is None:
+        v = workspace(nv * 4, x.device, "planes_v")
+    assert v.numel() >= nv and w.is_contiguous() and tuple(w.shape) == (Cout, Cin, 3, 3)
+    ws = workspace(lib().vd_conv3x3_wino43_fwd_planes_ws_bytes(nimg, H, W, Cin, Cout), x.device, "planes")
+    args = (ptr(x), ldx, ptr(w), ptr(bias), ptr(res), ldres, ptr(y), ldy, nimg, H, W, Cin, Cout, ptr(stats_part), ptr(v), ws.data_ptr(),
+            ws.numel() * 4)
+    phase = lambda ph: _check(lib().vd_conv3x3_wino43_fwd_planes(*args, ph, stream()), "vd_conv3x3_wino43_fwd_planes")
+    if PROFILE is None:
+        phase(7)
+        return
+    T = nimg * (H // 4) * (W // 4)
+    with _TimedBytes("wino43_wgrad_transform_kernel", 4.0 * nimg * H * W * Cin * (1 + 2.25)):
+        phase(1)
+    with _TimedTile("gemm_dma_kernel<{tile}, 0, 0, false, {kt}>", 2.0 * 36 * T * Cout * Cin):
+        phase(2)
+    _note_bytes(PROFILE[-1][0], 4.0 * 36.0 * (T * (Cin + Cout) + Cout * Cin))
+    with _TimedBytes("wino43_out_transform_kernel", 4.0 * (36.0 * T * Cout + nimg * H * W * Cout * (2 if res is not None else 1))):
+        phase(4)
+
+
 def conv3x3_dgrad_wino43(dy, lddy, U43, dx, lddx, nimg, H, W, Cin, Cout):
     with _TimedName(f"wino43_conv_kernel<{W // 4}, false>", 2.0 * nimg * H * W * Cout * 9 * Cin):
         _check(lib().vd_conv3x3_dgrad_wino43(ptr(dy), lddy, ptr(U43), ptr(dx), lddx, nimg, H, W, Cin, Cout, stream()),
@@ -495,23 +541,37 @@
             and bool(lib().vd_conv3x3_wgrad_wino43_supported(nimg, H, W, Cin, Cout, ldx, lddy)))
 
 
-def conv3x3_wgrad_wino43(x, ldx, dy, lddy, nimg, H, W, Cin, Cout, dw, Cin_w, Cout_w, accumulate=False, dbias=None):
+def conv3x3_wgrad_wino43(x, ldx, dy, lddy, nimg, H, W, Cin, Cout, dw, Cin_w, Cout_w, accumulate=False, dbias=None, v=None):
     nb = lib().vd_conv3x3_wgrad_wino43_ws_bytes(nimg, H, W, Cin, Cout)
-    ws = workspace(nb, x.device, "wgrad43")
-    args = _wgrad_args(x, ldx, dy, lddy, nimg, H, W, Cin, Cout, dw, dbias, Cin_w, Cout_w, accumulate, ws)
+    ws = workspace(nb, dy.device, "wgrad43")
+    if v is not None:
+        assert v.numel() == lib().vd_conv3x3_wino43_v_floats(nimg, H, W, Cin)
+        vargs = (ptr(v), ptr(dy), lddy, nimg, H, W, Cin, Cout, ptr(dw), ptr(dbias), Cin_w, Cout_w, int(accumulate), ws.data_ptr(),
+                 ws.numel() * 4)
+        phase = lambda ph: _check(lib().vd_conv3x3_wgrad_wino43_v(*vargs, ph, stream()), "vd_conv3x3_wgrad_wino43_v")
+    else:
+        args = _wgrad_args(x, ldx, dy, lddy, nimg, H, W, Cin, Cout, dw, dbias, Cin_w, Cout_w, accumulate, ws)
+        phase = lambda ph: _check(lib().vd_conv3x3_wgrad_wino43_phase(*args, ph, stream()), "vd_conv3x3_wgrad_wino43_phase")
     if PROFILE is None:
-        _check(lib().vd_conv3x3_wgrad_wino43(*args, stream()), "vd_conv3x3_wgrad_wino43")
+        if v is not None:
+            phase(7)
+        else:
+            _check(lib().vd_conv3x3_wgrad_wino43(*args, stream()), "vd_conv3x3_wgrad_wino43")
         return
-    with _TimedBytes("wino43_wgrad_transform_kernel", 4.0 * nimg * H * W * (Cin + Cout) * (1 + 2.25)):
-        _check(lib().vd_conv3x3_wgrad_wino43_phase(*args, 1, stream()), "vd_conv3x3_wgrad_wino43_phase")
+    with _TimedBytes("wino43_wgrad_transform_kernel", 4.0 * nimg * H * W * ((Cin if v is None else 0) + Cout) * (1 + 2.25)):
+        phase(1)
     with _TimedTile("gemm_dma_kernel<{tile}, 1, 1, true, {kt}, true> " + W43_WGRAD_TAG, 2.0 * nimg * H * W * Cout * 9 * Cin) as t:
-        _check(lib().vd_conv3x3_wgrad_wino43_phase(*args, 2, stream()), "vd_conv3x3_wgrad_wino43_phase")
+        phase(2)
     _note_bytes(PROFILE[-1][0], 4.0 * (36.0 * nimg * (H // 4) * (W // 4) * (Cin + Cout) + 36.0 * Cout * Cin))
     with _TimedName("wino43_wgrad_finish_kernel", 0.0):
-        _check(lib().vd_conv3x3_wgrad_wino43_phase(*args, 4, stream()), "vd_conv3x3_wgrad_wino43_phase")
-
-
-def conv3x3_wgrad(x, ldx, dy, lddy, nimg, H, W, Cin, Cout, dw, Cin_w, Cout_w, accumulate=False, dbias=None, direct=False):
+        phase(4)
+
+
+def conv3x3_wgrad(x, ldx, dy, lddy, nimg, H, W, Cin, Cout, dw, Cin_w, Cout_w, accumulate=False, dbias=None, direct=False, v=None):
+    if v is not None:
+        if direct or not wgrad43_supported(nimg, H, W, Cin, Cout, Cin, lddy):
+            raise HipError("conv3x3_wgrad: a V image was kept for a geometry the F(4x4,3x3) weight gradient does not serve")
+        return conv3x3_wgrad_wino43(None, Cin, dy, lddy, nimg, H, W, Cin, Cout, dw, Cin_w, Cout_w, accumulate, dbias, v=v)
     if not direct and wgrad43_supported(nimg, H, W, Cin, Cout, ldx, lddy):
         return conv3x3_wgrad_wino43(x, ldx, dy, lddy, nimg, H, W, Cin, Cout, dw, Cin_w, Cout_w, accumulate, dbias)
     if WINO and not direct and lib().vd_conv3x3_wgrad_wino_supported(nimg, H, W, Cin, Cout, ldx, lddy):
diff --git a/v-diffusion-torch_amd/v_diffusion/engine.py b/v-diffusion-torch_amd/v_diffusion/engine.py
--- a/v-diffusion-torch_amd/v_diffusion/engine.py
+++ b/v-diffusion-torch_amd/v_diffusion/engine.py
@@ -251,12 +251,14 @@
         if len(q) == H.GROUP_MAX:
             self._wgrad_flush_key(key)
 
-    def _cwgrad(self, x, ldx, dy, lddy, *args, **kw):
+    def _cwgrad(self, x, ldx, dy, lddy, *args, v=None, **kw):
+        if v is not None:
+            kw["v"] = v
         side = self._side
         if side is None:
             return H.conv3x3_wgrad(x, ldx, dy, lddy, *args, **kw)
         side.wait_stream(torch.cuda.current_stream())
-        x.record_stream(side)
+        (x if v is None else v).record_stream(side)
         dy.record_stream(side)
         with torch.cuda.stream(side):
             H.conv3x3_wgrad(x, ldx, dy, lddy, *args, **kw)
@@ -355,8 +357,16 @@
     def _layer(self, w):
         return self._packs.layers.get(id(w), _NO_PACK) if self._packs is not None else _NO_PACK
 
-    def _conv(self, x, ldx, w, bias, y, ldy, B, Hh, Ww, Cin, Cout, dgrad=False, res=None, ldres=0, stats_part=None):
+    def _conv(self, x, ldx, w, bias, y, ldy, B, Hh, Ww, Cin, Cout, dgrad=False, res=None, ldres=0, stats_part=None, keep_v=None):
         pk, p = self._packs, self._layer(w)
+        if not dgrad and p is not _NO_PACK and pk.wino and H.conv_planes_supported(B, Hh, Ww, Cin, Cout, ldx, ldy, ldres if res is not None else 0,
+                                                                                 training=keep_v is not None):
+            v = None
+            if keep_v is not None:
+                v = torch.empty(36 * B * (Hh // 4) * (Ww // 4) * Cin, dtype=torch.float32, device=x.device)
+                keep_v.append(v)
+            H.conv3x3_wino43_fwd_planes(x, ldx, w, bias, y, ldy, B, Hh, Ww, Cin, Cout, res=res, ldres=ldres, stats_part=stats_part, v=v)
+            return H.wino43_fwd_chunk_rows(Hh, Ww)
         if not dgrad and p.u43f is not None and H.wino43_fwd_supported(B, Hh, Ww, Cin, Cout, ldx, ldy, ldres if res is not None else 0):
             H.conv3x3_wino43_fwd(x, ldx, p.u43f, bias, y, ldy, B, Hh, Ww, Cin, Cout, res=res, ldres=ldres, stats_part=stats_part)
             return H.wino43_fwd_chunk_rows(Hh, Ww)
@@ -521,7 +531,8 @@
         coef1 = self._norm(x, x_parts, mod.norm1, None, 1, 0.0, 0, rs, a1, B, Hh, Ww, Cin)
         h1 = self._new(x, B, Ho, Wo, Cout)
         ph = self._part(x, B, Ho * Wo, Cout)
-        rows = self._conv(a1, Cin, mod.conv1.weight, mod.conv1.bias, h1, Cout, B, Ho, Wo, Cin, Cout, stats_part=ph)
+        v1, v2 = ([], []) if tape is not None else (None, None)
+        rows = self._conv(a1, Cin, mod.conv1.weight, mod.conv1.bias, h1, Cout, B, Ho, Wo, Cin, Cout, stats_part=ph, keep_v=v1)
         h1_parts = self._parts(ph, Cout, Ho * Wo, rows)
         c2, fi = blk.film
         film = films[c2][fi]
@@ -541,11 +552,11 @@
             sk = xs
         pd = self._part(x, B, Ho * Wo, Cout)
         rows = self._conv(a2, Cout, mod.conv2.weight, mod.conv2.bias, dest, _ld(dest), B, Ho, Wo, Cout, Cout, res=sk,
-                          ldres=_ld(sk), stats_part=pd)
+                          ldres=_ld(sk), stats_part=pd, keep_v=v2)
         out_parts = self._parts(pd, Cout, Ho * Wo, rows)
         if tape is not None:
-            tape[prefix] = dict(x=x, coef1=coef1, a1=a1, h1=h1, coef2=coef2, a2=a2, film=film, xs=xs if has_skip else None,
-                                seed=seed, p=p_drop)
+            tape[prefix] = dict(x=x, coef1=coef1, a1=None if v1 else a1, h1=h1, coef2=coef2, a2=None if v2 else a2, film=film,
+                                xs=xs if has_skip else None, seed=seed, p=p_drop, v1=v1[0] if v1 else None, v2=v2[0] if v2 else None)
         return out_parts
 
     def _res_bwd(self, blk, ctx, dy, dx, dx_accumulate, ta, dfilms, G):
@@ -555,7 +566,7 @@
         B, Hh, Ww, Cin, ldx = _chk(x)
         _, Ho, Wo, Cout, lddy = _chk(dy)
         rs = blk.rs
-        self._cwgrad(a2, Cout, dy, lddy, B, Ho, Wo, Cout, Cout, g["conv2.weight"], Cout, Cout, dbias=g["conv2.bias"])
+        self._cwgrad(a2, Cout, dy, lddy, B, Ho, Wo, Cout, Cout, g["conv2.weight"], Cout, Cout, dbias=g["conv2.bias"], v=ctx["v2"])
         da2 = self._new(x, B, Ho, Wo, Cout)
         self._conv(dy, lddy, mod.conv2.weight, None, da2, Cout, B, Ho, Wo, Cout, Cout, dgrad=True)
         dh1 = self._new(x, B, Ho, Wo, Cout)
@@ -565,7 +576,7 @@
                        H.RS_NONE, None, 0, dh1, Cout, False, dfilm, None, None, False, B, Ho, Wo, Cout, GROUPS,
                        pgb_keep=self._pgb(B, Cout, g["norm2.weight"], g["norm2.bias"]))
         del da2
-        self._cwgrad(a1, Cin, dh1, Cout, B, Ho, Wo, Cin, Cout, g["conv1.weight"], Cin, Cout, dbias=g["conv1.bias"])
+        self._cwgrad(a1, Cin, dh1, Cout, B, Ho, Wo, Cin, Cout, g["conv1.weight"], Cin, Cout, dbias=g["conv1.bias"], v=ctx["v1"])
         da1 = self._new(x, B, Ho, Wo, Cin)
         self._conv(dh1, Cout, mod.conv1.weight, None, da1, Cin, B, Ho, Wo, Cout, Cin, dgrad=True)
         del dh1
```
